# hlesmqh/WS3D

Measured on AMD Instinct MI355X. Metric: KITTI scenes/sec (16384 pts) Stage-1 RPN fwd, 1/2/4/8 GPU; FPS+group HBM GB/s, higher is better.
Workload: dtype f32

## Files before the change

include/ws3d_ops.h:

```cpp
#ifndef WS3D_OPS_H
#define WS3D_OPS_H

#include <stddef.h>
#include <stdint.h>

#ifdef __cplusplus
extern "C" {
#endif

#define WS3D_OK 0
#define WS3D_E_INVALID (-1)
#define WS3D_E_LAUNCH (-2)
#define WS3D_E_WORKSPACE (-3)
#define WS3D_E_UNSUPPORTED (-4)

#if defined(__GNUC__)
#define WS3D_API __attribute__((visibility("default")))
#else
#define WS3D_API
#endif

typedef void *ws3d_stream_t;

#define WS3D_ABI_VERSION 6
// ... 57 lines not shown
                  int32_t *idx, const void *sorted_known, ws3d_stream_t stream);

WS3D_API int ws3d_three_nn_weights(long rows, const float *dist2, float *weight, ws3d_stream_t stream);
WS3D_API int ws3d_three_nn_w(int b, int n, int m, const float *unknown, const float *known, float *dist2, int32_t *idx, float *weight,
                             const void *sorted_known, ws3d_stream_t stream);
WS3D_API int ws3d_three_nn_wq(int b, int n, int m, const float *unknown, const float *known, float *dist2, int32_t *idx, float *weight,
                              const void *sorted_known, const void *sorted_unknown, ws3d_stream_t stream);
WS3D_API int ws3d_three_nn_jobs(int b, int njobs, const int *n, const int *m, const float *const *unknown, const void *const *sorted_known,
                                float *const *dist2, int32_t *const *idx, float *const *weight, const void *const *sorted_unknown,
                                ws3d_stream_t stream);

WS3D_API int ws3d_pool_nsample(long rows, int nsample, const float *x, float *out, uint8_t *arg, ws3d_stream_t stream);
WS3D_API int ws3d_pool_nsample_grad(long rows, int nsample, const float *grad_out, const uint8_t *arg, float *grad_x,
                                    ws3d_stream_t stream);

WS3D_API int ws3d_gemm_pool(long rows, int nsample, int k_dim, int o_dim, const float *x_rows, const float *wt,
                            const float *bias, int relu, float *out, int out_stride, const int32_t *gate, long gate_limit, ws3d_stream_t stream);

WS3D_API int ws3d_gather_gemm(int b, int n, int m, int nsample, int c_feat, int o_dim, const float *feats, const float *xyz,
                     const float *new_xyz, const int32_t *nbr, const float *wt, const float *bias, int relu, float *out,
                     ws3d_stream_t stream);

WS3D_API int ws3d_gather_gemm2(int b, int n, int m, int nsample, int c_feat, int o1, int o2, const float *feats, const float *xyz,
                      const float *new_xyz, const int32_t *nbr, const float *w1t, const float *b1, int relu1, const float *w2t,
                      const float *b2, int relu2, float *out, ws3d_stream_t stream);

WS3D_API int ws3d_pgather_gemm2(int b, int n, int m, int nsample, int o1, int o2, const float *pmat, int p_stride, const float *xyz,
                       const float *new_xyz, const int32_t *nbr, const float *w1x, const float *b1, int relu1,
                       const float *w2t, const float *b2, int relu2, float *out, const int32_t *gate, long gate_limit, ws3d_stream_t stream);
WS3D_API int ws3d_pgather_rows(int b, int n, int m, int nsample, int o1, const float *pmat, int p_stride, const float *xyz, const float *new_xyz,
                      const int32_t *nbr, const float *w1x, const float *b1, int relu1, float *out, ws3d_stream_t stream);

WS3D_API int ws3d_qinterp_rows(int b, int n, int m, int o, const float *q, const int32_t *idx, const float *weight, const float *lin,
                      const float *skip, int c1, const float *wb, const float *bias, int relu, float *out, ws3d_stream_t stream);


WS3D_API int ws3d_compact_pairs(long centres, int nsample, const int32_t *nbr, int32_t *rowc, int32_t *rowsrc, int32_t *total, ws3d_stream_t stream);
WS3D_API int ws3d_compact_pairs_count(long centres, int nsample, const int32_t *nbr, int32_t *cnt, ws3d_stream_t stream);
WS3D_API int ws3d_compact_pairs_rows(long centres, int nsample, const int32_t *nbr, const int32_t *cnt, const int32_t *incl, int32_t *rowc,
                            int32_t *rowsrc, int32_t *total, ws3d_stream_t stream);
WS3D_API int ws3d_pgather_gemm2_compact(int b, int n, int m, long max_rows, int o1, int o2, const float *pmat, int p_stride, const float *xyz,
                               const float *new_xyz, const int32_t *rowc, const int32_t *rowsrc, const int32_t *total, const float *w1x,
                               const float *b1, int relu1, const float *w2t, const float *b2, int relu2, float *out, long limit, ws3d_stream_t stream);
WS3D_API int ws3d_pgather_gemm3_compact(int b, int n, int m, long max_rows, int o1, int o2, int o3, const float *pmat, int p_stride, const float *xyz,
                               const float *new_xyz, const int32_t *rowc, const int32_t *rowsrc, const int32_t *total, const float *w1x,
                               const float *b1, int relu1, const float *w2t, const float *b2, int relu2, const float *w3t, const float *b3,
                               float *out, int out_stride, long limit, ws3d_stream_t stream);
WS3D_API int ws3d_gemm_pool_compact(long max_rows, int k_dim, int o_dim, const float *x_rows, const int32_t *rowc, const int32_t *total,
                           const float *wt, const float *bias, float *out, int out_stride, long limit, ws3d_stream_t stream);
typedef struct ws3d_compact_mlp_args {
    int b, n, m;
    long max_rows;
    int o1, o2, o3;
    const float *pmat;
    int p_stride;
    const float *xyz, *new_xyz;
    const int32_t *rowc, *rowsrc, *total;
    const float *w1x, *b1;
    int relu1;
    const float *w2t, *b2;
    int relu2;
    const float *w3t, *b3;
    float *mid;
    float *out;
    int out_stride;
    long limit;
} ws3d_compact_mlp_args;
WS3D_API int ws3d_compact_mlp_pair(int kind, const ws3d_compact_mlp_args *scale0, const ws3d_compact_mlp_args *scale1, ws3d_stream_t stream);
WS3D_API int ws3d_chain_mlp3_ticket_ints(void);
WS3D_API size_t ws3d_chain_mlp3_blob_floats(int o2);
WS3D_API int ws3d_chain_mlp3_pack(const ws3d_compact_mlp_args *scale, float *blob, ws3d_stream_t stream);
WS3D_API int ws3d_chain_mlp3(const ws3d_compact_mlp_args *scale0, const ws3d_compact_mlp_args *scale1, const float *blob0, const float *blob1,
                             int32_t *ticket, int workgroups, ws3d_stream_t stream);

WS3D_API int ws3d_sa_mlp3_pool_compact(int b, int n, int m, long max_rows, int c1, int c2, int c3, const float *xyz, const float *new_xyz,
                              const float *feat, const int32_t *rowc, const int32_t *rowsrc, const int32_t *total, const float *w1t,
                              const float *b1, const float *w2t, const float *b2, const float *w3t, const float *b3, float *out,
                              int out_stride, long limit, ws3d_stream_t stream);

WS3D_API int ws3d_sa_mlp3_pool_lists(int b, int n, int m, int nsample, int c1, int c2, int c3, const float *xyz, const float *new_xyz,
                            const float *feat, const int32_t *nbr, const float *w1t, const float *b1, const float *w2t, const float *b2,
                            const float *w3t, const float *b3, int relu3, float *out, int out_stride, const int32_t *gate, long gate_limit,
                            ws3d_stream_t stream);

WS3D_API int ws3d_interp_gemm(int b, int n, int m, int c2, int c1, int o_dim, const float *known_feats, const float *unknown_feats,
                     const int32_t *idx, const float *weight, const float *wt, const float *bias, int relu, float *out,
                     ws3d_stream_t stream);

WS3D_API size_t ws3d_conv1x1_wgrad_workspace_bytes(int b, int o, int c, long l);
WS3D_API int ws3d_conv1x1_wgrad(int b, int o, int c, long l, const float *grad_out, const float *x, float *grad_w,
                                void *workspace, size_t workspace_bytes, ws3d_stream_t stream);

WS3D_API size_t ws3d_bn_workspace_bytes(int b, int c, long l);
WS3D_API int ws3d_bn_relu_train_fwd(int b, int c, long l, const float *x, const float *gamma, const float *beta, float eps,
                                    float momentum, int relu, float *running_mean, float *running_var,
                                    int64_t *num_batches_tracked, float *y, float *save_mean, float *save_invstd,
                                    void *workspace, size_t workspace_bytes, ws3d_stream_t stream);
WS3D_API int ws3d_bn_relu_train_bwd(int b, int c, long l, const float *x, const float *dy, const float *gamma,
                                    const float *beta, const float *save_mean, const float *save_invstd, int relu, float *dx,
                                    float *dgamma, float *dbeta, void *workspace, size_t workspace_bytes, ws3d_stream_t stream);

WS3D_API int ws3d_three_interpolate(int b, int c, int m, int n, const float *points, const int32_t *idx,
                           const float *weight, float *out, ws3d_stream_t stream);

WS3D_API int ws3d_three_interpolate_grad(int b, int c, int n, int m, const float *grad_out,
                                const int32_t *idx, const float *weight, float *grad_points,
                                ws3d_stream_t stream);

WS3D_API size_t ws3d_scatter_workspace_bytes(int b, int c, int n_targets, long slots_per_scene);
WS3D_API int ws3d_group_points_grad_det(int b, int c, int n, int npoints, int nsample, const float *grad_out,
                                        const int32_t *idx, float *grad_points, void *workspace,
                                        size_t workspace_bytes, ws3d_stream_t stream);
WS3D_API int ws3d_three_interpolate_grad_det(int b, int c, int n, int m, const float *grad_out, const int32_t *idx,
                                             const float *weight, float *grad_points, void *workspace,
                                             size_t workspace_bytes, ws3d_stream_t stream);

WS3D_API int ws3d_bias_act_inplace(int b, int o_ch, long l, int relu, float *y, const float *bias,
                                   ws3d_stream_t stream);

WS3D_API int ws3d_rowmax_bias_act(int b, int o_ch, long m, int s, int relu, const float *y, const float *bias,
                                  float *out, ws3d_stream_t stream);

WS3D_API int ws3d_query_and_group_nlc(int b, int n, int m, int c, float radius, int nsample, int use_xyz,
                                      const float *xyz, const float *new_xyz, const float *features_nlc,
                                      int32_t *idx_out, float *out_nlc, const void *sorted, ws3d_stream_t stream);
WS3D_API int ws3d_three_interpolate_nlc(int b, int c, int m, int n, const float *feats_nlc, const int32_t *idx,
                                        const float *weight, float *out_nlc, int out_stride, ws3d_stream_t stream);
WS3D_API int ws3d_rowmax_rows(long rows_out, int ns, int o_ch, const float *y, float *out, int out_stride,
                              ws3d_stream_t stream);

WS3D_API int ws3d_sa_mlp3_pool(long rows, int nsample, int c1, int c2, int c3, const float *x_rows4,
                               const float *w1t, const float *b1, const float *w2t, const float *b2,
                               const float *w3t, const float *b3, int relu3, float *out, int out_stride,
                               ws3d_stream_t stream);

WS3D_API int ws3d_mlp2_rows(long rows, int k_dim, int o1, int o2, const float *x_rows, const float *w1t, const float *b1, int relu1,
                   const float *w2t, const float *b2, int relu2, float *out, int *ticket, ws3d_stream_t stream);

WS3D_API size_t ws3d_rpn_heads_blob_bytes(int o2);
WS3D_API int ws3d_rpn_heads_pack(int o2, const float *w1t, const float *b1, int relu1, const float *w2t, const float *b2, int relu2, void *blob,
                        ws3d_stream_t stream);
WS3D_API int ws3d_rpn_heads(long rows, const float *x_rows, int heads, const void *blob_cls, float *out_cls, int *ticket_cls, int o2_reg,
                   const void *blob_reg, float *out_reg, int *ticket_reg, int workgroups, ws3d_stream_t stream);

WS3D_API size_t ws3d_gemm_rows_pack_bytes(int k_dim, int n_dim);
WS3D_API int ws3d_gemm_rows_pack(int k_dim, int n_dim, const float *wt, void *pack, ws3d_stream_t stream);
WS3D_API int ws3d_gemm_rows_split(long rows, int k_dim, int n_dim, const float *a, const void *pack, const float *bias, int relu, float *out,
                         ws3d_stream_t stream);

WS3D_API int ws3d_qinterp_gemm(int b, int n, int m, int c, int o_dim, const float *q, const int32_t *idx, const float *weight, const float *lin,
                      const float *skip, int c1, const float *wb, const float *b1, int relu1, const float *w2t, const float *b2, int relu2,
                      float *out, ws3d_stream_t stream);


WS3D_API int ws3d_boxes_overlap_bev(int num_a, const float *boxes_a, int num_b, const float *boxes_b,
                           float *ans, ws3d_stream_t stream);

WS3D_API int ws3d_boxes_iou_bev(int num_a, const float *boxes_a, int num_b, const float *boxes_b,
                       float *ans, ws3d_stream_t stream);

WS3D_API int ws3d_boxes_iou3d_paired(int n, const float *boxes_a, const float *boxes_b, float *overlap_bev, float *iou2d, float *iou3d,
                                     ws3d_stream_t stream);

WS3D_API int ws3d_nms_mask(int boxes_num, const float *boxes, float thresh, int normal, int full_grid,
                  uint64_t *mask, ws3d_stream_t stream);

WS3D_API size_t ws3d_nms_workspace_bytes(int boxes_num);
WS3D_API int ws3d_nms(int boxes_num, const float *boxes, float thresh, int normal, int max_keep,
                      void *workspace, size_t workspace_bytes, int64_t *keep, int32_t *num_keep,
                      ws3d_stream_t stream);

WS3D_API int ws3d_nms_batched(int batch, int boxes_num, const float *boxes, float thresh, int normal,
                              int max_keep, void *workspace, size_t workspace_bytes, int64_t *keep,
                              int32_t *num_keep, ws3d_stream_t stream);


WS3D_API int ws3d_radius_nms_batched(int batch, int n, const float *centers, float radius, int max_keep,
                                     void *workspace, size_t workspace_bytes, int64_t *keep,
                                     int32_t *num_keep, ws3d_stream_t stream);

WS3D_API int ws3d_topk_sorted(int b, int n, int k, const float *scores, float *out_scores, int64_t *out_idx,
                              ws3d_stream_t stream);
WS3D_API size_t ws3d_topk_workspace_bytes(int b, int n);
WS3D_API int ws3d_topk_sorted_ws(int b, int n, int k, const float *scores, float *out_scores, int64_t *out_idx, void *workspace,
                                 size_t workspace_bytes, ws3d_stream_t stream);
WS3D_API int ws3d_topk_sorted_sigmoid(int b, int n, int k, const float *logits, float *out_scores, int64_t *out_idx, ws3d_stream_t stream);
WS3D_API int ws3d_topk_sorted_sigmoid_ws(int b, int n, int k, const float *logits, float *out_scores, int64_t *out_idx, void *workspace,
                                         size_t workspace_bytes, ws3d_stream_t stream);

WS3D_API int ws3d_decode_center_boxes(int b, int n, int bins, float loc_scope, float loc_bin_size, float h, float w,
                                      float l, const float *xyz, const float *rpn_reg, float *boxes,
                                      ws3d_stream_t stream);

WS3D_API int ws3d_gather_boxes_bev(int b, int n, int top, const float *box, const int64_t *order, float *box_sorted, float *bev,
                          ws3d_stream_t stream);
WS3D_API int ws3d_decode_gather_boxes_bev(int b, int n, int top, int bins, float loc_scope, float loc_bin_size, float h, float w, float l,
                                          const float *xyz, const float *rpn_reg, const int64_t *order, float *box_sorted, float *bev,
                                          ws3d_stream_t stream);
WS3D_API int ws3d_select_proposals(int b, int top, int keep_stride, int k, const float *box_sorted, const float *scores_sorted,
                          const int64_t *keep, const int32_t *num, float extra_width, float *boxes_out, float *scores_out,
                          int64_t *count, float *pooled_boxes, ws3d_stream_t stream);
WS3D_API int ws3d_select_proposals_packed(int b, int top, int keep_stride, int k, const float *box_sorted, const float *scores_sorted,
                                          const int64_t *keep, const int32_t *num, float extra_width, float *boxes_out, float *scores_out,
                                          int64_t *count, float *pooled_boxes, float *packed, ws3d_stream_t stream);
WS3D_API int ws3d_select_proposals_send(int b, int top, int keep_stride, int k, const float *box_sorted, const float *scores_sorted,
                                        const int64_t *keep, const int32_t *num, float extra_width, float *boxes_out, float *scores_out,
                                        int64_t *count, float *pooled_boxes, float *send, long send_stride, ws3d_stream_t stream);
WS3D_API int ws3d_split_points_clear(long rows, int c, const float *pc, float *xyz, float *feats, void *clear, size_t clear_bytes,
                                     ws3d_stream_t stream);


WS3D_API int ws3d_roipool3d(int batch_size, int pts_num, int boxes_num, int feature_in_len,
                   int sampled_pts_num, const float *xyz, const float *boxes3d,
                   const float *pts_feature, float *pooled_features, int32_t *pooled_empty_flag,
                   int32_t *pts_idx, ws3d_stream_t stream);
WS3D_API int ws3d_roipool3d_fill(int batch_size, int pts_num, int boxes_num, int feature_in_len,
                   int sampled_pts_num, const float *xyz, const float *boxes3d,
                   const float *pts_feature, float *pooled_features, int32_t *pooled_empty_flag,
                   int32_t *pts_idx, ws3d_stream_t stream);

WS3D_API size_t ws3d_roipool3d_workspace_bytes(int batch_size, int pts_num);
WS3D_API int ws3d_roipool3d_ws(int batch_size, int pts_num, int boxes_num, int feature_in_len, int sampled_pts_num, const float *xyz,
                               const float *boxes3d, const float *pts_feature, float *pooled_features, int32_t *pooled_empty_flag,
                               int32_t *pts_idx, int fill, void *workspace, size_t workspace_bytes, ws3d_stream_t stream);


WS3D_API int ws3d_pts_in_boxes3d(int boxes_num, int pts_num, const float *pts, const float *boxes3d,
                        int64_t *flag, ws3d_stream_t stream);


WS3D_API int ws3d_instance_clouds(int batch, int pts_num, int centres_num, int feat_len, int sampled_pts_num, float radius, int mask_mode,
                                  float mask_thresh, const float *pts, const float *score, const float *feats, const float *centres,
                                  const int32_t *num, float *cloud, float *cloud_feats, int32_t *count, int32_t *pts_idx,
                                  ws3d_stream_t stream);
WS3D_API int ws3d_instance_clouds_count(int batch, int pts_num, int centres_num, float radius, const float *pts, const float *centres,
                                        const int32_t *num, int32_t *count, ws3d_stream_t stream);
WS3D_API int ws3d_instance_clouds_emit(int batch, int pts_num, int centres_num, int feat_len, float radius, int mask_mode, float mask_thresh,
                                       const float *pts, const float *score, const float *feats, const float *centres, const int32_t *num,
                                       const int64_t *offsets, float *rows, float *row_feats, int32_t *row_idx, ws3d_stream_t stream);


WS3D_API int ws3d_click_prepare(int batch, int pts_num, int clicks_num, int side, const float *offsets, float gauss_height, float gauss_status,
                                float gauss_cov, float centre_y, const float *pts, const float *clicks, const int32_t *num, float *score,
                                float *cand, int32_t *cand_num, ws3d_stream_t stream);



WS3D_API int ws3d_kitti_overlaps(int metric, int criterion, int frames, long max_pairs, const int32_t *gt_off, const int32_t *dt_off,
                                 const int64_t *out_off, const double *dt_boxes, const double *gt_boxes, double *out,
                                 ws3d_stream_t stream);

WS3D_API int ws3d_kitti_collect_scores(int frames, int max_dt, const int32_t *gt_off, const int32_t *dt_off, const int64_t *out_off,
                                       const double *overlaps, const int32_t *ignored_gt, const int32_t *ignored_dt,
                                       const double *dt_score, double min_overlap, double *tp_score, int32_t *tp_flag,
                                       ws3d_stream_t stream);

WS3D_API size_t ws3d_kitti_count_workspace_bytes(int frames, int num_thresh);
WS3D_API int ws3d_kitti_count(int metric, int frames, int max_dt, int num_thresh, const double *thresholds, const int32_t *gt_off,
                              const int32_t *dt_off, const int32_t *dc_off, const int64_t *out_off, const double *overlaps,
                              const int32_t *ignored_gt, const int32_t *ignored_dt, const double *dt_score, const double *dt_alpha,
                              const double *gt_alpha, const double *dt_bbox, const double *dc_bbox, double min_overlap, int compute_aos,
                              void *workspace, size_t workspace_bytes, double *pr, ws3d_stream_t stream);


WS3D_API int ws3d_stage2_embed(long rows, int pts_per_cloud, const float *pts, const float *box_ce, float extend, const float *wx0,
                               const float *bx0, const float *wx1, const float *bx1, const float *wf0, const float *bf0, const float *wf1,
                               const float *bf1, const float *wm, const float *bm, float *xyz_out, float *feat, ws3d_stream_t stream);
WS3D_API int ws3d_stage2_boxes(int rows, int loc_bins, int head_bins, float loc_scope, float h, float w, float l, const float *rcnn_reg,
                               float *pred_boxes3d, float *box_ce, ws3d_stream_t stream);
WS3D_API int ws3d_stage2_select(int batch, int slots, float cls_thresh, float iou_thresh, const float *size_window, float ground_y,
                                const float *box_ce, const float *rcnn_ref, const float *rcnn_cls, const float *rcnn_iou, const float *center,
                                const int32_t *num, float *boxes, int32_t *keep, float *key, ws3d_stream_t stream);

WS3D_API int ws3d_stage2_rcnn_loss(int rows, int loc_bins, int head_bins, float loc_scope, float h, float w, float l, const float *rcnn_cls,
                                   const float *rcnn_reg, const float *pred_boxes3d, const float *gt_boxes, const float *cls, float *vals,
                                   int32_t *counts, float *grad_cls, float *grad_reg, ws3d_stream_t stream);
WS3D_API int ws3d_stage2_ioun_loss(int rows, const float *rcnn_iou, const float *rcnn_ref, const float *pred_boxes3d, const float *refined_box,
                                   const float *gt_boxes, const float *cls, float *vals, int32_t *counts, float *grad_iou, float *grad_ref,
                                   ws3d_stream_t stream);

WS3D_API int ws3d_rpn_center_labels(int batch, int n, int kmax, int pts_stride, float gauss_height, float gauss_status, double gauss_cov,
                                    const float *pts, const float *centres, const int32_t *count, float *cls_label, float *reg_label,
                                    ws3d_stream_t stream);
WS3D_API size_t ws3d_rpn_loss_workspace_bytes(int rows);
WS3D_API int ws3d_rpn_loss(int rows, int bins, double loc_scope, double loc_bin_size, double alpha, double gamma, double weight_cls,
                           double weight_reg, const float *rpn_cls, const float *rpn_reg, const float *cls_label, const float *reg_label,
                           float *vals, int32_t *counts, float *grad_cls, float *grad_reg, void *workspace, size_t workspace_bytes,
                           ws3d_stream_t stream);

#ifdef __cplusplus
}
#endif
#endif
```

ws3d_amd/_lib.py:

```python
from __future__ import annotations

import ctypes as C
import os

_HERE = os.path.dirname(os.path.abspath(__file__))
DIST_MODE = int(os.environ.get("WS3D_DIST_MODE", "0") or 0)
LIB_PATH = os.environ.get("WS3D_HIP_LIB") or os.path.join(
    _HERE, "libws3d_hip.so" if DIST_MODE == 0 else "libws3d_hip_dm%d.so" % DIST_MODE)

E_INVALID, E_LAUNCH, E_WORKSPACE, E_UNSUPPORTED = -1, -2, -3, -4
ABI_VERSION = 6

_vp = C.c_void_p
_i = C.c_int
_f = C.c_float
_sz = C.c_size_t

class CompactMlpArgs(C.Structure):
    _fields_ = [("b", _i), ("n", _i), ("m", _i), ("max_rows", C.c_long), ("o1", _i), ("o2", _i), ("o3", _i), ("pmat", _vp), ("p_stride", _i),
                ("xyz", _vp), ("new_xyz", _vp), ("rowc", _vp), ("rowsrc", _vp), ("total", _vp), ("w1x", _vp), ("b1", _vp), ("relu1", _i),
                ("w2t", _vp), ("b2", _vp), ("relu2", _i), ("w3t", _vp), ("b3", _vp), ("mid", _vp), ("out", _vp), ("out_stride", _i), ("limit", C.c_long)]


SIGNATURES = {
    "ws3d_abi_version": (_i, []),
    "ws3d_tune": (_i, [_i, _i]),
    "ws3d_dist_mode": (_i, []),
    "ws3d_last_error": (C.c_char_p, []),
    "ws3d_device_info": (_i, [C.c_char_p, _i, C.POINTER(_i), C.POINTER(_i)]),
    "ws3d_furthest_point_sampling": (_i, [_i, _i, _i, _vp, _vp, _vp, _vp]),
    "ws3d_furthest_point_sampling_gather": (_i, [_i, _i, _i, _vp, _vp, _vp, _vp, _vp]),
    "ws3d_furthest_point_sampling_nested": (_i, [_i, _i, _i, _vp, _vp, _vp, _vp]),
    "ws3d_furthest_point_sampling_nested_chain": (_i, [_i, _i, _i, _vp, _vp, _vp, _vp, _vp]),
    "ws3d_gather_points": (_i, [_i, _i, _i, _i, _vp, _vp, _vp, _vp]),
    "ws3d_gather_points_grad": (_i, [_i, _i, _i, _i, _vp, _vp, _vp, _vp]),
    "ws3d_ball_query": (_i, [_i, _i, _i, _f, _i, _vp, _vp, _vp, _vp, _vp]),
    "ws3d_ball_query_fill": (_i, [_i, _i, _i, _f, _i, _vp, _vp, _vp, _vp, _vp]),
    "ws3d_ball_query_pairs": (_i, [_i, _i, _i, _f, _i, _vp, _vp, _vp, _vp, _vp, _vp, _vp, _vp]),
    "ws3d_ball_query_pairs2": (_i, [_i, _i, _i, _vp, _vp, _vp, C.c_float, _i, _vp, _vp, _vp, _vp, C.c_float, _i, _vp, _vp, _vp, _vp, _vp]),
    "ws3d_sorted_points_bytes": (_sz, [_i, _i]),
    "ws3d_sort_points_x": (_i, [_i, _i, _vp, _vp, _vp]),
    "ws3d_sort_points_xz": (_i, [_i, _i, _vp, _vp, _vp]),
    "ws3d_sort_points_grid": (_i, [_i, _i, _vp, _vp, _vp]),
    "ws3d_sort_points_jobs": (_i, [_i, _i, _vp, _vp, _vp, _vp, _vp]),
    "ws3d_group_points": (_i, [_i, _i, _i, _i, _i, _vp, _vp, _vp, _vp]),
    "ws3d_group_points_grad": (_i, [_i, _i, _i, _i, _i, _vp, _vp, _vp, _vp]),
    "ws3d_query_and_group": (_i, [_i, _i, _i, _i, _f, _i, _i, _vp, _vp, _vp, _vp, _vp, _vp, _vp]),
    "ws3d_three_nn": (_i, [_i, _i, _i, _vp, _vp, _vp, _vp, _vp, _vp]),
    "ws3d_three_interpolate": (_i, [_i, _i, _i, _i, _vp, _vp, _vp, _vp, _vp]),
    "ws3d_three_interpolate_grad": (_i, [_i, _i, _i, _i, _vp, _vp, _vp, _vp, _vp]),
    "ws3d_bn_workspace_bytes": (C.c_size_t, [_i, _i, C.c_long]),
    "ws3d_bn_relu_train_fwd": (_i, [_i, _i, C.c_long, _vp, _vp, _vp, C.c_float, C.c_float, _i, _vp, _vp, _vp, _vp, _vp, _vp,
                                    _vp, C.c_size_t, _vp]),
    "ws3d_bn_relu_train_bwd": (_i, [_i, _i, C.c_long, _vp, _vp, _vp, _vp, _vp, _vp, _i, _vp, _vp, _vp, _vp, C.c_size_t, _vp]),
    "ws3d_conv1x1_wgrad_workspace_bytes": (C.c_size_t, [_i, _i, _i, C.c_long]),
    "ws3d_conv1x1_wgrad": (_i, [_i, _i, _i, C.c_long, _vp, _vp, _vp, _vp, C.c_size_t, _vp]),
    "ws3d_gemm_pool": (_i, [C.c_long, _i, _i, _i, _vp, _vp, _vp, _i, _vp, _i, _vp, C.c_long, _vp]),
    "ws3d_pool_nsample": (_i, [C.c_long, _i, _vp, _vp, _vp, _vp]),
    "ws3d_pool_nsample_grad": (_i, [C.c_long, _i, _vp, _vp, _vp, _vp]),
    "ws3d_scatter_workspace_bytes": (C.c_size_t, [_i, _i, _i, C.c_long]),
    "ws3d_group_points_grad_det": (_i, [_i, _i, _i, _i, _i, _vp, _vp, _vp, _vp, C.c_size_t, _vp]),
    "ws3d_three_interpolate_grad_det": (_i, [_i, _i, _i, _i, _vp, _vp, _vp, _vp, _vp, C.c_size_t, _vp]),
    "ws3d_query_and_group_nlc": (_i, [_i, _i, _i, _i, _f, _i, _i, _vp, _vp, _vp, _vp, _vp, _vp, _vp]),
    "ws3d_three_interpolate_nlc": (_i, [_i, _i, _i, _i, _vp, _vp, _vp, _vp, _i, _vp]),
    "ws3d_rowmax_rows": (_i, [C.c_long, _i, _i, _vp, _vp, _i, _vp]),
    "ws3d_sa_mlp3_pool": (_i, [C.c_long, _i, _i, _i, _i, _vp, _vp, _vp, _vp, _vp, _vp, _vp, _i, _vp, _i, _vp]),
    "ws3d_qinterp_gemm": (_i, [_i, _i, _i, _i, _i, _vp, _vp, _vp, _vp, _vp, _i, _vp, _vp, _i, _vp, _vp, _i, _vp, _vp]),
    "ws3d_mlp2_rows": (_i, [C.c_long, _i, _i, _i, _vp, _vp, _vp, _i, _vp, _vp, _i, _vp, _vp, _vp]),
    "ws3d_rpn_heads_blob_bytes": (_sz, [_i]),
    "ws3d_rpn_heads_pack": (_i, [_i, _vp, _vp, _i, _vp, _vp, _i, _vp, _vp]),
    "ws3d_rpn_heads": (_i, [C.c_long, _vp, _i, _vp, _vp, _vp, _i, _vp, _vp, _vp, _i, _vp]),
    "ws3d_gemm_rows_pack_bytes": (_sz, [_i, _i]),
    "ws3d_gemm_rows_pack": (_i, [_i, _i, _vp, _vp, _vp]),
    "ws3d_gemm_rows_split": (_i, [C.c_long, _i, _i, _vp, _vp, _vp, _i, _vp, _vp]),
    "ws3d_decode_center_boxes": (_i, [_i, _i, _i, _f, _f, _f, _f, _f, _vp, _vp, _vp, _vp]),
    "ws3d_topk_sorted": (_i, [_i, _i, _i, _vp, _vp, _vp, _vp]),
    "ws3d_topk_workspace_bytes": (C.c_size_t, [_i, _i]),
    "ws3d_topk_sorted_ws": (_i, [_i, _i, _i, _vp, _vp, _vp, _vp, C.c_size_t, _vp]),
    "ws3d_topk_sorted_sigmoid": (_i, [_i, _i, _i, _vp, _vp, _vp, _vp]),
    "ws3d_topk_sorted_sigmoid_ws": (_i, [_i, _i, _i, _vp, _vp, _vp, _vp, C.c_size_t, _vp]),
    "ws3d_three_nn_weights": (_i, [C.c_long, _vp, _vp, _vp]),
    "ws3d_three_nn_w": (_i, [_i, _i, _i, _vp, _vp, _vp, _vp, _vp, _vp, _vp]),
    "ws3d_three_nn_wq": (_i, [_i, _i, _i, _vp, _vp, _vp, _vp, _vp, _vp, _vp, _vp]),
    "ws3d_three_nn_jobs": (_i, [_i, _i, _vp, _vp, _vp, _vp, _vp, _vp, _vp, _vp, _vp]),
    "ws3d_bias_act_inplace": (_i, [_i, _i, C.c_long, _i, _vp, _vp, _vp]),
    "ws3d_rowmax_bias_act": (_i, [_i, _i, C.c_long, _i, _i, _vp, _vp, _vp, _vp]),
    "ws3d_boxes_overlap_bev": (_i, [_i, _vp, _i, _vp, _vp, _vp]),
    "ws3d_boxes_iou_bev": (_i, [_i, _vp, _i, _vp, _vp, _vp]),
    "ws3d_boxes_iou3d_paired": (_i, [_i, _vp, _vp, _vp, _vp, _vp, _vp]),
    "ws3d_nms_mask": (_i, [_i, _vp, _f, _i, _i, _vp, _vp]),
    "ws3d_nms_workspace_bytes": (_sz, [_i]),
    "ws3d_nms": (_i, [_i, _vp, _f, _i, _i, _vp, _sz, _vp, _vp, _vp]),
    "ws3d_nms_batched": (_i, [_i, _i, _vp, _f, _i, _i, _vp, _sz, _vp, _vp, _vp]),
    "ws3d_radius_nms_batched": (_i, [_i, _i, _vp, _f, _i, _vp, _sz, _vp, _vp, _vp]),
    "ws3d_gather_gemm": (_i, [_i, _i, _i, _i, _i, _i, _vp, _vp, _vp, _vp, _vp, _vp, _i, _vp, _vp]),
    "ws3d_gather_gemm2": (_i, [_i, _i, _i, _i, _i, _i, _i, _vp, _vp, _vp, _vp, _vp, _vp, _i, _vp, _vp, _i, _vp, _vp]),
    "ws3d_pgather_gemm2": (_i, [_i, _i, _i, _i, _i, _i, _vp, _i, _vp, _vp, _vp, _vp, _vp, _i, _vp, _vp, _i, _vp, _vp, C.c_long, _vp]),
    "ws3d_pgather_rows": (_i, [_i, _i, _i, _i, _i, _vp, _i, _vp, _vp, _vp, _vp, _vp, _i, _vp, _vp]),
    "ws3d_qinterp_rows": (_i, [_i, _i, _i, _i, _vp, _vp, _vp, _vp, _vp, _i, _vp, _vp, _i, _vp, _vp]),
    "ws3d_compact_pairs": (_i, [C.c_long, _i, _vp, _vp, _vp, _vp, _vp]),
    "ws3d_compact_pairs_count": (_i, [C.c_long, _i, _vp, _vp, _vp]),
    "ws3d_compact_pairs_rows": (_i, [C.c_long, _i, _vp, _vp, _vp, _vp, _vp, _vp, _vp]),
    "ws3d_pgather_gemm2_compact": (_i, [_i, _i, _i, C.c_long, _i, _i, _vp, _i, _vp, _vp, _vp, _vp, _vp, _vp, _vp, _i, _vp, _vp, _i, _vp, C.c_long, _vp]),
    "ws3d_pgather_gemm3_compact": (_i, [_i, _i, _i, C.c_long, _i, _i, _i, _vp, _i, _vp, _vp, _vp, _vp, _vp, _vp, _vp, _i, _vp, _vp, _i, _vp, _vp, _vp, _i, C.c_long, _vp]),
    "ws3d_gemm_pool_compact": (_i, [C.c_long, _i, _i, _vp, _vp, _vp, _vp, _vp, _vp, _i, C.c_long, _vp]),
    "ws3d_compact_mlp_pair": (_i, [_i, C.POINTER(CompactMlpArgs), C.POINTER(CompactMlpArgs), _vp]),
    "ws3d_chain_mlp3_ticket_ints": (_i, []),
    "ws3d_chain_mlp3_blob_floats": (_sz, [_i]),
    "ws3d_chain_mlp3_pack": (_i, [C.POINTER(CompactMlpArgs), _vp, _vp]),
    "ws3d_chain_mlp3": (_i, [C.POINTER(CompactMlpArgs), C.POINTER(CompactMlpArgs), _vp, _vp, _vp, _i, _vp]),
    "ws3d_sa_mlp3_pool_compact": (_i, [_i, _i, _i, C.c_long, _i, _i, _i, _vp, _vp, _vp, _vp, _vp, _vp, _vp, _vp, _vp, _vp, _vp, _vp, _vp, _i, C.c_long, _vp]),
    "ws3d_sa_mlp3_pool_lists": (_i, [_i, _i, _i, _i, _i, _i, _i, _vp, _vp, _vp, _vp, _vp, _vp, _vp, _vp, _vp, _vp, _i, _vp, _i, _vp, C.c_long, _vp]),
    "ws3d_interp_gemm": (_i, [_i, _i, _i, _i, _i, _i, _vp, _vp, _vp, _vp, _vp, _vp, _i, _vp, _vp]),
    "ws3d_gather_boxes_bev": (_i, [_i, _i, _i, _vp, _vp, _vp, _vp, _vp]),
    "ws3d_select_proposals": (_i, [_i, _i, _i, _i, _vp, _vp, _vp, _vp, _f, _vp, _vp, _vp, _vp, _vp]),
    "ws3d_decode_gather_boxes_bev": (_i, [_i, _i, _i, _i, _f, _f, _f, _f, _f, _vp, _vp, _vp, _vp, _vp, _vp]),
    "ws3d_select_proposals_packed": (_i, [_i, _i, _i, _i, _vp, _vp, _vp, _vp, _f, _vp, _vp, _vp, _vp, _vp, _vp]),
    "ws3d_select_proposals_send": (_i, [_i, _i, _i, _i, _vp, _vp, _vp, _vp, _f, _vp, _vp, _vp, _vp, _vp, C.c_long, _vp]),
    "ws3d_split_points_clear": (_i, [C.c_long, _i, _vp, _vp, _vp, _vp, C.c_size_t, _vp]),
    "ws3d_roipool3d": (_i, [_i, _i, _i, _i, _i, _vp, _vp, _vp, _vp, _vp, _vp, _vp]),
    "ws3d_roipool3d_fill": (_i, [_i, _i, _i, _i, _i, _vp, _vp, _vp, _vp, _vp, _vp, _vp]),
    "ws3d_roipool3d_workspace_bytes": (C.c_size_t, [_i, _i]),
    "ws3d_roipool3d_ws": (_i, [_i, _i, _i, _i, _i, _vp, _vp, _vp, _vp, _vp, _vp, _i, _vp, C.c_size_t, _vp]),
    "ws3d_pts_in_boxes3d": (_i, [_i, _i, _vp, _vp, _vp, _vp]),
    "ws3d_instance_clouds": (_i, [_i, _i, _i, _i, _i, _f, _i, _f, _vp, _vp, _vp, _vp, _vp, _vp, _vp, _vp, _vp, _vp]),
    "ws3d_instance_clouds_count": (_i, [_i, _i, _i, _f, _vp, _vp, _vp, _vp, _vp]),
    "ws3d_instance_clouds_emit": (_i, [_i, _i, _i, _i, _f, _i, _f, _vp, _vp, _vp, _vp, _vp, _vp, _vp, _vp, _vp, _vp]),
    "ws3d_click_prepare": (_i, [_i, _i, _i, _i, _vp, _f, _f, _f, _f, _vp, _vp, _vp, _vp, _vp, _vp, _vp]),
    "ws3d_kitti_overlaps": (_i, [_i, _i, _i, C.c_long, _vp, _vp, _vp, _vp, _vp, _vp, _vp]),
    "ws3d_kitti_collect_scores": (_i, [_i, _i, _vp, _vp, _vp, _vp, _vp, _vp, _vp, C.c_double, _vp, _vp, _vp]),
    "ws3d_kitti_count_workspace_bytes": (_sz, [_i, _i]),
    "ws3d_kitti_count": (_i, [_i, _i, _i, _i, _vp, _vp, _vp, _vp, _vp, _vp, _vp, _vp, _vp, _vp, _vp, _vp, _vp, C.c_double, _i, _vp,
                              _sz, _vp, _vp]),
    "ws3d_stage2_embed": (_i, [C.c_long, _i, _vp, _vp, _f] + [_vp] * 10 + [_vp, _vp, _vp]),
    "ws3d_stage2_boxes": (_i, [_i, _i, _i, _f, _f, _f, _f, _vp, _vp, _vp, _vp]),
    "ws3d_stage2_select": (_i, [_i, _i, _f, _f, C.POINTER(_f), _f, _vp, _vp, _vp, _vp, _vp, _vp, _vp, _vp, _vp, _vp]),
    "ws3d_stage2_rcnn_loss": (_i, [_i, _i, _i, _f, _f, _f, _f] + [_vp] * 9 + [_vp]),
    "ws3d_stage2_ioun_loss": (_i, [_i] + [_vp] * 10 + [_vp]),
    "ws3d_rpn_center_labels": (_i, [_i, _i, _i, _i, _f, _f, C.c_double] + [_vp] * 5 + [_vp]),
    "ws3d_rpn_loss_workspace_bytes": (_sz, [_i]),
    "ws3d_rpn_loss": (_i, [_i, _i] + [C.c_double] * 6 + [_vp] * 8 + [_vp, _sz, _vp]),
}


class Ws3dError(RuntimeError):
    pass


_lib = None


def load() -> C.CDLL:
    global _lib
    if _lib is not None:
        return _lib
    if not os.path.exists(LIB_PATH):
        raise Ws3dError(
            f"{LIB_PATH} is missing: the MI355X HIP library has not been built "
            "(run `python -m ws3d_amd.build`).  ws3d_amd has no CPU fallback.")
    import torch
    try:
        lib = C.CDLL(LIB_PATH)
    except OSError as e:
        raise Ws3dError(f"cannot load {LIB_PATH}: {e}") from e
    for name, (res, args) in SIGNATURES.items():
        fn = getattr(lib, name)
        fn.restype = res
        fn.argtypes = args
    if lib.ws3d_abi_version() != ABI_VERSION:
        raise Ws3dError(f"{LIB_PATH} exports ABI version {lib.ws3d_abi_version()}, this package binds version {ABI_VERSION}: "
                        "rebuild it (`python -m ws3d_amd.build`)")
    if not os.environ.get("WS3D_HIP_LIB") and lib.ws3d_dist_mode() != DIST_MODE:
        raise Ws3dError(f"{LIB_PATH} was built with WS3D_DIST_MODE={lib.ws3d_dist_mode()}, expected {DIST_MODE}: rebuild it")
    _lib = lib
    return lib


def check(rc: int, what: str = "") -> None:
    if rc != 0:
        msg = load().ws3d_last_error()
        raise Ws3dError(f"{what or 'ws3d'} failed (rc={rc}): {msg.decode() if msg else ''}")
```

ws3d_amd/build.py:

```python
from __future__ import annotations

import argparse
import concurrent.futures as cf
import glob
import os
import shutil
import subprocess
import sys

HERE = os.path.dirname(os.path.abspath(__file__))
CSRC = os.path.join(HERE, "csrc")
OBJ = os.path.join(CSRC, "build")
LIB = os.path.join(HERE, "libws3d_hip.so")
DIST_MODES = (0, 1, 2)


def lib_path(dist_mode: int = 0) -> str:
    return LIB if dist_mode == 0 else os.path.join(HERE, "libws3d_hip_dm%d.so" % dist_mode)
ARCH = "gfx950"
SOURCES = ["core.hip", "fps.hip", "fps_v3.hip", "fps_bucket.hip", "fps_nested.hip", "ballquery_group.hip", "interpolate.hip", "roipool3d.hip", "iou3d.hip", "proposals.hip", "scatter_det.hip", "sa_mlp.hip", "bn_relu.hip", "gemm_pool.hip", "conv_wgrad.hip", "chain_mlp.hip", "rpn_heads.hip", "gemm_rows.hip", "kitti_eval.hip", "instance_clouds.hip", "click.hip", "stage2.hip", "stage2_loss.hip", "rpn_targets.hip"]
CXXFLAGS = ["-O3", "-std=c++17", "-fPIC", "-ffp-contract=off", "-fno-fast-math",
            "-fvisibility=hidden", "-Wall", "-Wno-unused-function"]


def hipcc() -> str:
    for cand in (os.environ.get("HIPCC"), shutil.which("hipcc"), "/opt/rocm/bin/hipcc"):
        if cand and os.path.exists(cand):
            return cand
    raise RuntimeError("hipcc not found (looked at $HIPCC, PATH, /opt/rocm/bin)")


def _deps(src: str):
    return [src, *glob.glob(os.path.join(CSRC, "*.h")), os.path.join(HERE, "..", "include", "ws3d_ops.h"),
            os.path.join(CSRC, "exports.map"), os.path.abspath(__file__)]


def _compile(src: str, force: bool, verbose: bool, dist_mode: int = 0) -> str:
    path = os.path.join(CSRC, src)
    obj = os.path.join(OBJ if dist_mode == 0 else OBJ + "_dm%d" % dist_mode, os.path.splitext(src)[0] + ".o")
    if not force and os.path.exists(obj) and all(
            os.path.getmtime(obj) >= os.path.getmtime(d) for d in _deps(path)):
        return obj
    cmd = [hipcc(), f"--offload-arch={ARCH}", *CXXFLAGS, f"-DWS3D_DIST_MODE={dist_mode}", *os.environ.get("WS3D_EXTRA_DEFS", "").split(), "-c", path, "-o", obj]
    if verbose:
        print(" ".join(cmd), flush=True)
    r = subprocess.run(cmd, capture_output=True, text=True)
    if r.returncode != 0:
        raise RuntimeError(f"hipcc failed for {src}:\n{r.stdout}\n{r.stderr}")
    if verbose and r.stderr.strip():
        print(r.stderr)
    return obj


def build(force: bool = False, verbose: bool = False, dist_mode: int = 0) -> str:
    LIB = lib_path(dist_mode)
    os.makedirs(OBJ if dist_mode == 0 else OBJ + "_dm%d" % dist_mode, exist_ok=True)
    with cf.ThreadPoolExecutor(max_workers=min(len(SOURCES), os.cpu_count() or 4, 16)) as ex:
        objs = list(ex.map(lambda s: _compile(s, force, verbose, dist_mode), SOURCES))
    if force or not os.path.exists(LIB) or any(os.path.getmtime(o) > os.path.getmtime(LIB) for o in objs):
        cmd = [hipcc(), f"--offload-arch={ARCH}", "-shared", "-fPIC", "-Wl,--version-script=" + os.path.join(CSRC, "exports.map"), "-o", LIB, *objs]
        if verbose:
            print(" ".join(cmd), flush=True)
        r = subprocess.run(cmd, capture_output=True, text=True)
        if r.returncode != 0:
            raise RuntimeError(f"link failed:\n{r.stdout}\n{r.stderr}")
    return LIB


def rebuild_one(src: str, verbose: bool = False) -> str:
    _compile(src, True, verbose)
    objs = [os.path.join(OBJ, os.path.splitext(s_)[0] + ".o") for s_ in SOURCES]
    missing = [o for o in objs if not os.path.exists(o)]
    if missing:
        return build(False, verbose)
    cmd = [hipcc(), f"--offload-arch={ARCH}", "-shared", "-fPIC", "-Wl,--version-script=" + os.path.join(CSRC, "exports.map"), "-o", LIB, *objs]
    r = subprocess.run(cmd, capture_output=True, text=True)
    if r.returncode != 0:
        raise RuntimeError(f"link failed:\n{r.stdout}\n{r.stderr}")
    return LIB


if __name__ == "__main__":
    ap = argparse.ArgumentParser()
    ap.add_argument("--force", action="store_true")
    ap.add_argument("--verbose", action="store_true")
    ap.add_argument("--dist-mode", type=int, default=0, choices=DIST_MODES)
    ap.add_argument("--all-dist-modes", action="store_true")
    ap.add_argument("--only", default=None, help="recompile this one source (forced) and relink")
    a = ap.parse_args()
    if a.only:
        print(rebuild_one(a.only, a.verbose))
        sys.exit(0)
    for dm in (DIST_MODES if a.all_dist_modes else (a.dist_mode,)):
        print(build(a.force, a.verbose, dm))
    sys.exit(0)
```

ws3d_amd/compat.py:

```python
from __future__ import annotations

import sys
import types

import os

import torch

from . import _lib
from ._lib import Ws3dError, check


def _dev(*tensors):
    dev = None
    for t in tensors:
        if t is None:
            continue
        if not t.is_cuda:
            raise Ws3dError("ws3d_amd ops need HIP ('cuda') tensors; there is no CPU fallback")
        if not t.is_contiguous():
            raise Ws3dError("ws3d_amd ops need contiguous tensors (the reference asserts the same)")
        if dev is None:
            dev = t.device
        elif t.device != dev:
# ... 355 lines not shown
    b, c = x.size(0), x.size(1)
    l = x.numel() // max(b * c, 1)
    y = torch.empty_like(x)
    mean = torch.empty((c,), dtype=torch.float32, device=dev)
    invstd = torch.empty((c,), dtype=torch.float32, device=dev)
    lib = _lib.load()
    nbytes = lib.ws3d_bn_workspace_bytes(b, c, l)
    ws = torch.empty((nbytes + 7) // 8, dtype=torch.float64, device=dev)
    with _on(dev):
        check(lib.ws3d_bn_relu_train_fwd(b, c, l, _p(x), _p(gamma), _p(beta), float(eps), float(momentum), int(bool(relu)),
                                         _p(running_mean), _p(running_var), _p(num_batches_tracked), _p(y), _p(mean), _p(invstd), _p(ws), nbytes,
                                         _stream()), "bn_relu_train_fwd")
    return y, mean, invstd


def bn_relu_train_bwd(x, dy, gamma, beta, save_mean, save_invstd, relu=True):
    dev = _dev(x, dy, gamma, beta, save_mean, save_invstd)
    _f32(x, "x"); _f32(dy, "dy")
    b, c = x.size(0), x.size(1)
    l = x.numel() // max(b * c, 1)
    dx = torch.empty_like(x)
    dgamma = torch.empty((c,), dtype=torch.float32, device=dev)
    dbeta = torch.empty((c,), dtype=torch.float32, device=dev)
    lib = _lib.load()
    nbytes = lib.ws3d_bn_workspace_bytes(b, c, l)
    ws = torch.empty((nbytes + 7) // 8, dtype=torch.float64, device=dev)
    with _on(dev):
        check(lib.ws3d_bn_relu_train_bwd(b, c, l, _p(x), _p(dy), _p(gamma), _p(beta), _p(save_mean), _p(save_invstd),
                                         int(bool(relu)), _p(dx), _p(dgamma), _p(dbeta), _p(ws), nbytes, _stream()),
              "bn_relu_train_bwd")
    return dx, dgamma, dbeta


def conv1x1_wgrad(grad_out, x, shape=None):
    dev = _dev(grad_out, x)
    _f32(grad_out, "grad_out"); _f32(x, "x")
    b, o, c = x.size(0), grad_out.size(1), x.size(1)
    l = x.numel() // max(b * c, 1)
    if grad_out.numel() != b * o * l:
        raise Ws3dError("conv1x1_wgrad: grad_out and x disagree in shape")
    gw = torch.empty((o, c) if shape is None else tuple(shape), dtype=torch.float32, device=dev)
    lib = _lib.load()
    nbytes = lib.ws3d_conv1x1_wgrad_workspace_bytes(b, o, c, l)
    ws = torch.empty((nbytes + 3) // 4, dtype=torch.float32, device=dev)
    with _on(dev):
        check(lib.ws3d_conv1x1_wgrad(b, o, c, l, _p(grad_out), _p(x), _p(gw), _p(ws), nbytes, _stream()), "conv1x1_wgrad")
    return gw


def _gate(gate):
    if gate is None:
        return None, 0
    total, limit = gate
    return total.data_ptr(), int(limit)


def gemm_pool(x_rows, wt, bias, relu, nsample, out, col0=0, gate=None):
    dev = _dev(x_rows, wt, bias)
    _f32(x_rows, "x_rows"); _f32(wt, "wt")
    rows, k = x_rows.shape
    o = wt.size(1)
    if rows % 64 or rows // 64 > 65535 or o % 64 or k % 4 or nsample not in (16, 32) or wt.size(0) != k:
        return False
    view = out[:, col0:col0 + o]
    with _on(dev):
        check(_lib.load().ws3d_gemm_pool(rows, nsample, k, o, _p(x_rows), _p(wt), _p(bias), int(bool(relu)), view.data_ptr(),
                                         out.size(1), *_gate(gate), _stream()), "gemm_pool")
    return True


def gather_gemm(feats, xyz, new_xyz, nbr, wt_feat_then_xyz, bias, relu):
    dev = _dev(feats, xyz, new_xyz, nbr, wt_feat_then_xyz)
    _f32(feats, "feats"); _f32(xyz, "xyz"); _f32(new_xyz, "new_xyz"); _i32(nbr, "nbr"); _f32(wt_feat_then_xyz, "wt")
    B, N, C = feats.shape
    M, ns = nbr.size(1), nbr.size(2)
    O = wt_feat_then_xyz.size(1)
    rows = B * M * ns
    if C % 4 or O % 64 or rows % 64 or rows // 64 > 65535 or wt_feat_then_xyz.size(0) != C + 3 or not feats.is_contiguous():
        return None
    out = torch.empty((rows, O), dtype=torch.float32, device=dev)
    with _on(dev):
        check(_lib.load().ws3d_gather_gemm(B, N, M, ns, C, O, _p(feats), _p(xyz), _p(new_xyz), _p(nbr), _p(wt_feat_then_xyz), _p(bias),
                                           int(bool(relu)), _p(out), _stream()), "gather_gemm")
    return out


def gather_gemm2(feats, xyz, new_xyz, nbr, w1t_feat_then_xyz, b1, relu1, w2t, b2, relu2):
    dev = _dev(feats, xyz, new_xyz, nbr, w1t_feat_then_xyz, w2t)
    _f32(feats, "feats"); _f32(xyz, "xyz"); _f32(new_xyz, "new_xyz"); _i32(nbr, "nbr"); _f32(w1t_feat_then_xyz, "w1t"); _f32(w2t, "w2t")
    B, N, C = feats.shape
    M, ns = nbr.size(1), nbr.size(2)
    O1, O2 = w1t_feat_then_xyz.size(1), w2t.size(1)
    rows = B * M * ns
    if (C % 4 or O1 not in (64, 128, 256) or O2 % 4 or rows % 64 or w1t_feat_then_xyz.size(0) != C + 3 or w2t.size(0) != O1 or
            not feats.is_contiguous() or not w2t.is_contiguous() or not w1t_feat_then_xyz.is_contiguous()):
        return None
    out = torch.empty((rows, O2), dtype=torch.float32, device=dev)
    with _on(dev):
        check(_lib.load().ws3d_gather_gemm2(B, N, M, ns, C, O1, O2, _p(feats), _p(xyz), _p(new_xyz), _p(nbr), _p(w1t_feat_then_xyz), _p(b1),
                                            int(bool(relu1)), _p(w2t), _p(b2), int(bool(relu2)), _p(out), _stream()), "gather_gemm2")
    return out


def pgather_gemm2(pmat, col0, o1, xyz, new_xyz, nbr, w1x, b1, relu1, w2t, b2, relu2, out=None, gate=None):
    dev = _dev(pmat, xyz, new_xyz, nbr, w1x, w2t)
    _f32(pmat, "pmat"); _f32(xyz, "xyz"); _f32(new_xyz, "new_xyz"); _i32(nbr, "nbr"); _f32(w1x, "w1x"); _f32(w2t, "w2t")
    B, N = xyz.size(0), xyz.size(1)
    M, ns = nbr.size(1), nbr.size(2)
    O2 = w2t.size(1)
    if (o1 not in (64, 128) or O2 % 4 or (M * ns) % 64 or pmat.dim() != 2 or pmat.size(0) != B * N or pmat.stride(1) != 1 or
            col0 < 0 or col0 + o1 > pmat.size(1) or tuple(w1x.shape) != (3, o1) or w2t.size(0) != o1 or not w1x.is_contiguous() or not w2t.is_contiguous()):
        return None
    if out is None:
        out = torch.empty((B * M * ns, O2), dtype=torch.float32, device=dev)
    elif tuple(out.shape) != (B * M * ns, O2) or not out.is_contiguous():
        raise ValueError("pgather_gemm2: out must be a contiguous (B*M*ns, O2) tensor")
    with _on(dev):
        check(_lib.load().ws3d_pgather_gemm2(B, N, M, ns, o1, O2, pmat.data_ptr() + 4 * col0, pmat.stride(0), _p(xyz), _p(new_xyz), _p(nbr), _p(w1x), _p(b1),
                                             int(bool(relu1)), _p(w2t), _p(b2), int(bool(relu2)), _p(out), *_gate(gate), _stream()), "pgather_gemm2")
    return out


def pgather_rows(pmat, col0, o1, xyz, new_xyz, nbr, w1x, b1, relu1):
    dev = _dev(pmat, xyz, new_xyz, nbr, w1x)
    _f32(pmat, "pmat"); _f32(xyz, "xyz"); _f32(new_xyz, "new_xyz"); _i32(nbr, "nbr"); _f32(w1x, "w1x")
    B, N = xyz.size(0), xyz.size(1)
    M, ns = nbr.size(1), nbr.size(2)
    if (o1 % 4 or col0 % 4 or pmat.dim() != 2 or pmat.size(0) != B * N or pmat.stride(1) != 1 or pmat.stride(0) % 4 or col0 < 0 or
            col0 + o1 > pmat.size(1) or tuple(w1x.shape) != (3, o1) or not w1x.is_contiguous() or pmat.data_ptr() % 16):
        return None
    out = torch.empty((B * M * ns, o1), dtype=torch.float32, device=dev)
    with _on(dev):
        check(_lib.load().ws3d_pgather_rows(B, N, M, ns, o1, pmat.data_ptr() + 4 * col0, pmat.stride(0), _p(xyz), _p(new_xyz), _p(nbr), _p(w1x), _p(b1),
                                            int(bool(relu1)), _p(out), _stream()), "pgather_rows")
    return out


def qinterp_rows(q, idx, weight, lin=None, skip=None, wb=None, bias=None, relu=True):
    dev = _dev(q, idx, weight)
    _f32(q, "q"); _i32(idx, "idx"); _f32(weight, "weight")
    B, M, O = q.shape
    N = idx.size(1)
    c1 = 0 if skip is None else skip.size(2)
    if (O % 4 or not q.is_contiguous() or (lin is None and c1 > 4) or (lin is not None and (tuple(lin.shape) != (B * N, O) or not lin.is_contiguous())) or
            (lin is None and c1 > 0 and (wb is None or tuple(wb.shape) != (c1, O) or not wb.is_contiguous() or not skip.is_contiguous()))):
        return None
    out = torch.empty((B * N, O), dtype=torch.float32, device=dev)
    with _on(dev):
        check(_lib.load().ws3d_qinterp_rows(B, N, M, O, _p(q), _p(idx), _p(weight), _p(lin), _p(skip), c1, _p(wb), _p(bias), int(bool(relu)), _p(out),
                                            _stream()), "qinterp_rows")
    return out


def qinterp_gemm(q, idx, weight, w2t, b2, relu2, lin=None, skip=None, wb=None, bias=None, relu=True):
    dev = _dev(q, idx, weight, w2t)
    _f32(q, "q"); _i32(idx, "idx"); _f32(weight, "weight"); _f32(w2t, "w2t")
    B, M, C = q.shape
    N = idx.size(1)
    O = w2t.size(1)
    c1 = 0 if skip is None else skip.size(2)
    if ((B * N) % 64 or C % 16 or O % 128 or w2t.size(0) != C or not q.is_contiguous() or not w2t.is_contiguous() or not idx.is_contiguous() or
            not weight.is_contiguous() or (lin is None and c1 > 4) or (lin is not None and (tuple(lin.shape) != (B * N, C) or not lin.is_contiguous())) or
            (lin is None and c1 > 0 and (wb is None or tuple(wb.shape) != (c1, C) or not wb.is_contiguous() or not skip.is_contiguous()))):
        return None
    out = torch.empty((B * N, O), dtype=torch.float32, device=dev)
    with _on(dev):
        check(_lib.load().ws3d_qinterp_gemm(B, N, M, C, O, _p(q), _p(idx), _p(weight), _p(lin), _p(skip), c1, _p(wb), _p(bias), int(bool(relu)), _p(w2t),
                                            _p(b2), int(bool(relu2)), _p(out), _stream()), "qinterp_gemm")
    return out


def compact_pairs(nbr, ordered=False):
    if not ordered:
        dev = _dev(nbr)
        _i32(nbr, "nbr")
        B, M, ns = nbr.shape
        rowc = torch.empty(B * M * ns, dtype=torch.int32, device=dev)
        rowsrc = torch.empty(B * M * ns, dtype=torch.int32, device=dev)
        total = torch.zeros(1, dtype=torch.int32, device=dev)
        with _on(dev):
            check(_lib.load().ws3d_compact_pairs(B * M, ns, _p(nbr), _p(rowc), _p(rowsrc), _p(total), _stream()), "compact_pairs")
        return rowc, rowsrc, total
    dev = _dev(nbr)
    _i32(nbr, "nbr")
    B, M, ns = nbr.shape
    centres = B * M
    cnt = torch.empty(centres, dtype=torch.int32, device=dev)
    rowc = torch.empty(centres * ns, dtype=torch.int32, device=dev)
    rowsrc = torch.empty(centres * ns, dtype=torch.int32, device=dev)
    total = torch.empty(1, dtype=torch.int32, device=dev)
    with _on(dev):
        lib = _lib.load()
        check(lib.ws3d_compact_pairs_count(centres, ns, _p(nbr), _p(cnt), _stream()), "compact_pairs_count")
        incl = torch.cumsum(cnt, dim=0, dtype=torch.int32)
        check(lib.ws3d_compact_pairs_rows(centres, ns, _p(nbr), _p(cnt), _p(incl), _p(rowc), _p(rowsrc), _p(total), _stream()), "compact_pairs_rows")
    return rowc, rowsrc, total


def pgather_gemm2_compact(pmat, col0, o1, xyz, new_xyz, pairs, w1x, b1, relu1, w2t, b2, relu2, limit=-1):
    rowc, rowsrc, total = pairs
    dev = _dev(pmat, xyz, new_xyz, rowc, w1x, w2t)
    _f32(pmat, "pmat"); _f32(xyz, "xyz"); _f32(new_xyz, "new_xyz"); _f32(w1x, "w1x"); _f32(w2t, "w2t")
    B, N = xyz.size(0), xyz.size(1)
    M = new_xyz.size(1)
    O2 = w2t.size(1)
    rows = rowc.numel()
    if (o1 not in (64, 128, 256) or O2 % 4 or pmat.dim() != 2 or pmat.size(0) != B * N or pmat.stride(1) != 1 or col0 < 0 or col0 + o1 > pmat.size(1) or
            tuple(w1x.shape) != (3, o1) or w2t.size(0) != o1 or not w1x.is_contiguous() or not w2t.is_contiguous()):
        return None
    out = torch.empty((rows, O2), dtype=torch.float32, device=dev)
    with _on(dev):
        check(_lib.load().ws3d_pgather_gemm2_compact(B, N, M, rows, o1, O2, pmat.data_ptr() + 4 * col0, pmat.stride(0), _p(xyz), _p(new_xyz), _p(rowc),
                                                     _p(rowsrc), _p(total), _p(w1x), _p(b1), int(bool(relu1)), _p(w2t), _p(b2), int(bool(relu2)), _p(out),
                                                     int(limit), _stream()), "pgather_gemm2_compact")
    return out


def pgather_gemm3_compact(pmat, col0, o1, xyz, new_xyz, pairs, w1x, b1, relu1, w2t, b2, relu2, w3t, b3, out2d, col_offset, limit=-1, max_lds=160 * 1024):
    rowc, rowsrc, total = pairs
    dev = _dev(pmat, xyz, new_xyz, rowc, w1x, w2t, w3t, out2d)
    _f32(pmat, "pmat"); _f32(xyz, "xyz"); _f32(new_xyz, "new_xyz"); _f32(w1x, "w1x"); _f32(w2t, "w2t"); _f32(w3t, "w3t"); _f32(out2d, "out2d")
    B, N = xyz.size(0), xyz.size(1)
    M = new_xyz.size(1)
    O2, O3 = w2t.size(1), w3t.size(1)
    rows = rowc.numel()
    lds = 4 * ((o1 + (O2 + 15) // 16 * 16) * 65 + 2 * 16 * 64)
    if (o1 not in (64, 128) or O2 % 4 or O3 % 128 or lds > min(max_lds, 160 * 1024 - 1024) or pmat.dim() != 2 or pmat.size(0) != B * N or pmat.stride(1) != 1 or
            col0 < 0 or col0 + o1 > pmat.size(1) or tuple(w1x.shape) != (3, o1) or w2t.size(0) != o1 or w3t.size(0) != O2 or not w1x.is_contiguous() or
            not w2t.is_contiguous() or not w3t.is_contiguous() or out2d.dim() != 2 or out2d.stride(1) != 1 or col_offset < 0 or col_offset + O3 > out2d.size(1)):
        return False
    with _on(dev):
        check(_lib.load().ws3d_pgather_gemm3_compact(B, N, M, rows, o1, O2, O3, pmat.data_ptr() + 4 * col0, pmat.stride(0), _p(xyz), _p(new_xyz), _p(rowc),
                                                     _p(rowsrc), _p(total), _p(w1x), _p(b1), int(bool(relu1)), _p(w2t), _p(b2), int(bool(relu2)), _p(w3t), _p(b3),
                                                     out2d.data_ptr() + 4 * col_offset, out2d.stride(0), int(limit), _stream()), "pgather_gemm3_compact")
    return True


def gemm_pool_compact(x_rows, pairs, wt, bias, out2d, col_offset, limit=-1):
    rowc, rowsrc, total = pairs
    dev = _dev(x_rows, rowc, wt, out2d)
    _f32(x_rows, "x_rows"); _f32(wt, "wt"); _f32(out2d, "out2d")
    rows, k = x_rows.shape
    o = wt.size(1)
    if (k % 4 or o % 64 or wt.size(0) != k or rows != rowc.numel() or not x_rows.is_contiguous() or not wt.is_contiguous() or out2d.dim() != 2 or
            out2d.stride(1) != 1 or col_offset < 0 or col_offset + o > out2d.size(1)):
        return False
    with _on(dev):
        check(_lib.load().ws3d_gemm_pool_compact(rows, k, o, _p(x_rows), _p(rowc), _p(total), _p(wt), _p(bias), out2d.data_ptr() + 4 * col_offset,
                                                 out2d.stride(0), int(limit), _stream()), "gemm_pool_compact")
    return True


def compact_mlp_pair(kind, scales, max_lds=160 * 1024, mids=None):
    import ctypes as C
    if len(scales) != 2 or scales[0]["o1"] != scales[1]["o1"]:
        return None if kind == 2 else False
    blocks, keep, outs = [], [], []
    for si, a in enumerate(scales):
        rowc, rowsrc, total = a["pairs"]
        pmat, xyz, new_xyz, w1x, w2t, w3t, out2d, o1, col0, col = a["pmat"], a["xyz"], a["new_xyz"], a["w1x"], a["w2t"], a["w3t"], a["out2d"], a["o1"], a["col0"], a["col_offset"]
        dev = _dev(pmat, xyz, new_xyz, rowc, w1x, w2t, w3t, out2d)
        for t_, nm in ((pmat, "pmat"), (xyz, "xyz"), (new_xyz, "new_xyz"), (w1x, "w1x"), (w2t, "w2t"), (w3t, "w3t"), (out2d, "out2d")):
            _f32(t_, nm)
        B, N, M = xyz.size(0), xyz.size(1), new_xyz.size(1)
        O2, O3 = w2t.size(1), w3t.size(1)
        rows = rowc.numel()
        lds3 = 4 * ((o1 + (O2 + 15) // 16 * 16) * 65 + 2 * 16 * 64)
        ok = (O2 % 4 == 0 and pmat.dim() == 2 and pmat.size(0) == B * N and pmat.stride(1) == 1 and col0 >= 0 and col0 + o1 <= pmat.size(1) and
              tuple(w1x.shape) == (3, o1) and w2t.size(0) == o1 and w3t.size(0) == O2 and w1x.is_contiguous() and w2t.is_contiguous() and w3t.is_contiguous() and
              out2d.dim() == 2 and out2d.stride(1) == 1 and col >= 0 and col + O3 <= out2d.size(1))
        if kind == 3:
            ok = ok and o1 in (64, 128) and O3 % 128 == 0 and lds3 <= min(max_lds, 160 * 1024 - 1024)
        elif kind == 2:
            ok = ok and o1 in (64, 128, 256)
        else:
            ok = ok and O3 % 64 == 0 and mids is not None and tuple(mids[si].shape) == (rows, O2) and mids[si].is_contiguous()
        if not ok:
            return None if kind == 2 else False
        mid = mids[si] if kind == 1 else (torch.empty((rows, O2), dtype=torch.float32, device=dev) if kind == 2 else None)
        outs.append(mid)
        keep.append((pmat, xyz, new_xyz, rowc, rowsrc, total, w1x, w2t, w3t, out2d, mid, a["b1"], a["b2"], a["b3"]))
        blocks.append(_lib.CompactMlpArgs(B, N, M, rows, o1, O2, O3, pmat.data_ptr() + 4 * col0, pmat.stride(0), _p(xyz), _p(new_xyz), _p(rowc), _p(rowsrc),
                                          _p(total), _p(w1x), _p(a["b1"]), int(bool(a["relu1"])), _p(w2t), _p(a["b2"]), int(bool(a["relu2"])), _p(w3t), _p(a["b3"]),
                                          _p(mid), out2d.data_ptr() + 4 * col, out2d.stride(0), -1))
    with _on(dev):
        rc = _lib.load().ws3d_compact_mlp_pair(int(kind), C.byref(blocks[0]), C.byref(blocks[1]), _stream())
    if rc == _lib.E_UNSUPPORTED:
        return None if kind == 2 else False
    check(rc, "compact_mlp_pair")
    return outs if kind == 2 else True


CHAIN_WORKGROUPS = 0
TUNE_KEYS = {"chain_wgs": 0, "mlp2_wgs": 1, "sa1_wgs": 2, "fp_wgs": 3, "pair_wgs": 4, "bq_wide_nw": 5}


def tune(name: str, value: int = -1) -> int:
    rc = _lib.load().ws3d_tune(TUNE_KEYS[name], int(value))
    if rc < 0:
        check(rc, "tune")
    return rc


_CHAIN_BLOBS = {}


def chain_ticket_ints() -> int:
    return int(_lib.load().ws3d_chain_mlp3_ticket_ints())


def _chain_blob(block, tensors, dev):
    import ctypes as C
    key = tuple((t.data_ptr(), t._version) if t is not None else None for t in tensors)
    hit = _CHAIN_BLOBS.get(key)
    if hit is None:
        n = int(_lib.load().ws3d_chain_mlp3_blob_floats(block.o2))
        blob = torch.empty(n, dtype=torch.float32, device=dev)
        with _on(dev):
            check(_lib.load().ws3d_chain_mlp3_pack(C.byref(block), _p(blob), _stream()), "chain_mlp3_pack")
# ... 898 lines not shown
```

ws3d_amd/csrc/gemm_pool.hip:

```cpp
#include <cstdlib>

#include "common.h"
#include "compact_pool.h"
#include "mfma_tile.h"

namespace ws3d {

template <int NS, int MB, int NB>
__global__ __launch_bounds__(256) void gemm_pool_big_kernel(int k_dim, int o_dim, const float *__restrict__ x,
                                                            const float *__restrict__ wt, const float *__restrict__ bias,
                                                            int relu, float *__restrict__ out, int out_stride, int xcd,
                                                            const int32_t *__restrict__ gate, long gate_limit) {
    if (gate && (long)*gate <= gate_limit) return;
    constexpr int TM = 64 * MB, TN = 64 * NB;
    __shared__ float xs[2][GP_KT][TM + 1];
    __shared__ __attribute__((aligned(16))) float ws[2][GP_KT][TN];
    const Wave w;
    long row_tile;
    int col_tile;
    gg_tile<false>(o_dim / TN, xcd, blockIdx.x, row_tile, col_tile);
    const long row0 = row_tile * TM;
    const int col0 = col_tile * TN;
    RowsA<MB> load_a;
    load_a.k_dim = k_dim;
#pragma unroll
    for (int i = 0; i < MB; ++i) load_a.p[i] = x + (row0 + (w.tid >> 2) + 64 * i) * (long)k_dim;
    floatx16 acc[MB][NB];
    mfma_k_loop<MB, NB, false>(w, acc, xs, ws, k_dim, load_a, wt, o_dim, col0);
#pragma unroll
    for (int i = 0; i < MB; ++i)
#pragma unroll
        for (int j = 0; j < NB; ++j)
            pool_rows<NS>(w, acc[i][j], bias, relu, out, out_stride, row0 + sub_row<MB>(w, i), col0 + sub_col<NB, false>(w, j) + w.l32);
}

struct GatherA {
    const float *frow, *prow, *crow;
    int c_feat;
    __device__ __forceinline__ GatherA(long r, int c_feat_, int n, int m, int ns, const float *__restrict__ feats, const float *__restrict__ xyz,
                                       const float *__restrict__ new_xyz, const int32_t *__restrict__ nbr) {
        const long cm = r / ns;
        const long b = cm / m;
        const int src = nbr[r];
        frow = feats + ((size_t)b * n + (size_t)src) * c_feat_;
        prow = xyz + ((size_t)b * n + (size_t)src) * 3;
        crow = new_xyz + (size_t)cm * 3;
        c_feat = c_feat_;
    }
    __device__ __forceinline__ float4 operator()(int, int k) const {
        if (k < c_feat) return *reinterpret_cast<const float4 *>(frow + k);
        if (k == c_feat) return make_float4(prow[0] - crow[0], prow[1] - crow[1], prow[2] - crow[2], 0.f);
        return f4_zero();
    }
};

__global__ __launch_bounds__(256) void gather_gemm_kernel(int c_feat, int o_dim, int n, int m, int ns, const float *__restrict__ feats,
                                                          const float *__restrict__ xyz, const float *__restrict__ new_xyz,
                                                          const int32_t *__restrict__ nbr, const float *__restrict__ wt,
                                                          const float *__restrict__ bias, int relu, float *__restrict__ out, int tps) {
    __shared__ float xs[2][GP_KT][GP_XS];
    __shared__ __attribute__((aligned(16))) float ws[2][GP_KT][64];
    const Wave w;
    long row_tile;
    int col_tile;
    gg_tile<true>(o_dim / 64, tps, blockIdx.x, row_tile, col_tile);
    const long row0 = row_tile * 64;
    const int col0 = col_tile * 64;
    const GatherA load_a(row0 + (w.tid >> 2), c_feat, n, m, ns, feats, xyz, new_xyz, nbr);
    floatx16 acc[1][1];
    mfma_k_loop<1, 1, false>(w, acc, xs, ws, c_feat + 3, load_a, wt, o_dim, col0);
    store_rows(w, acc[0][0], bias, relu, out, o_dim, row0 + w.wm * 32, col0 + w.bc);
}

template <int NB1>
__global__ __launch_bounds__(256) void gather_gemm2_kernel(int c_feat, int o2, int n, int m, int ns, const float *__restrict__ feats,
                                                           const float *__restrict__ xyz, const float *__restrict__ new_xyz,
                                                           const int32_t *__restrict__ nbr, const float *__restrict__ w1t,
                                                           const float *__restrict__ b1, int relu1, const float *__restrict__ w2t,
                                                           const float *__restrict__ b2, int relu2, float *__restrict__ out) {
    constexpr int O1 = NB1 * 64;
    extern __shared__ __attribute__((aligned(16))) float smem2[];
    auto &xs = *reinterpret_cast<float (*)[2][GP_KT][GP_XS]>(smem2);
    auto &w1s = *reinterpret_cast<float (*)[2][GP_KT][O1]>(smem2 + 2 * GP_KT * GP_XS);
    float *act = smem2, *w2s = smem2 + O1 * GP_XS;
    const Wave w;
    const long row0 = (long)blockIdx.x * 64;
    const GatherA load_a(row0 + (w.tid >> 2), c_feat, n, m, ns, feats, xyz, new_xyz, nbr);
    floatx16 acc1[1][NB1];
    mfma_k_loop<1, NB1, true>(w, acc1, xs, w1s, c_feat + 3, load_a, w1t, O1, 0);
#pragma unroll
    for (int j = 0; j < NB1; ++j) store_act(w, acc1[0][j], b1, relu1, act, j * 64 + w.bc);
    lds_layer<1>(w, act, O1 / GP_KT, w2t, O1, o2, w2s, 0, 1, [&](const floatx16 &acc, int col) __attribute__((always_inline)) {
        if (col < o2) store_rows(w, acc, b2, relu2, out, o2, row0 + w.wm * 32, col);
    });
}

template <int NB1>
__global__ __launch_bounds__(256) void pgather_gemm2_kernel(int o2, int n, int m, int ns, const float *__restrict__ pmat, int p_stride,
                                                            const float *__restrict__ xyz, const float *__restrict__ new_xyz,
                                                            const int32_t *__restrict__ nbr, const float *__restrict__ w1x,
                                                            const float *__restrict__ b1, int relu1, const float *__restrict__ w2t,
                                                            const float *__restrict__ b2, int relu2, float *__restrict__ out,
                                                            const int32_t *__restrict__ gate, long gate_limit) {
    if (gate && (long)*gate <= gate_limit) return;
    constexpr int O1 = NB1 * 64;
    extern __shared__ __attribute__((aligned(16))) float smem2[];
    float *act = smem2, *w2s = smem2 + O1 * GP_XS;
    const Wave w;
    const long row0 = (long)blockIdx.x * 64;
    const long scene = row0 / ((long)m * ns);
    ppoint_layer1<NB1>(w, [&](int tr) __attribute__((always_inline)) { return PairRow{scene, (row0 + tr) / ns, nbr[row0 + tr]}; }, n, pmat, p_stride, xyz, new_xyz, w1x, b1, relu1, act);
    lds_layer<1>(w, act, O1 / GP_KT, w2t, O1, o2, w2s, 0, 1, [&](const floatx16 &acc, int col) __attribute__((always_inline)) {
        if (col < o2) store_rows(w, acc, b2, relu2, out, o2, row0 + w.wm * 32, col);
    });
}

__global__ __launch_bounds__(256) void pgather_rows_kernel(long rows, int o1, int n, int m, int ns, const float *__restrict__ pmat, int p_stride,
                                                           const float *__restrict__ xyz, const float *__restrict__ new_xyz,
                                                           const int32_t *__restrict__ nbr, const float *__restrict__ w1x,
                                                           const float *__restrict__ b1, int relu1, float *__restrict__ out) {
    const int q4 = o1 >> 2;
    const long total = rows * q4;
    for (long e = (long)blockIdx.x * 256 + threadIdx.x; e < total; e += (long)gridDim.x * 256) {
        const long r = e / q4;
        const int c4 = (int)(e - r * q4) * 4;
        const long cm = r / ns, scene = cm / m;
        const int src = nbr[r];
        const float *pr = xyz + ((size_t)scene * n + (size_t)src) * 3, *cr = new_xyz + (size_t)cm * 3;
        const float dx = pr[0] - cr[0], dy = pr[1] - cr[1], dz = pr[2] - cr[2];
        const float4 pv = *reinterpret_cast<const float4 *>(pmat + ((size_t)scene * n + (size_t)src) * p_stride + c4);
        const float4 wx = *reinterpret_cast<const float4 *>(w1x + c4), wy = *reinterpret_cast<const float4 *>(w1x + o1 + c4),
                     wz = *reinterpret_cast<const float4 *>(w1x + 2 * o1 + c4);
        const float4 bv = b1 ? *reinterpret_cast<const float4 *>(b1 + c4) : make_float4(0.f, 0.f, 0.f, 0.f);
        float4 y;
        y.x = __builtin_fmaf(dz, wz.x, __builtin_fmaf(dy, wy.x, __builtin_fmaf(dx, wx.x, pv.x))) + bv.x;
        y.y = __builtin_fmaf(dz, wz.y, __builtin_fmaf(dy, wy.y, __builtin_fmaf(dx, wx.y, pv.y))) + bv.y;
        y.z = __builtin_fmaf(dz, wz.z, __builtin_fmaf(dy, wy.z, __builtin_fmaf(dx, wx.z, pv.z))) + bv.z;
        y.w = __builtin_fmaf(dz, wz.w, __builtin_fmaf(dy, wy.w, __builtin_fmaf(dx, wx.w, pv.w))) + bv.w;
        if (relu1) { y.x = y.x < 0.f ? 0.f : y.x; y.y = y.y < 0.f ? 0.f : y.y; y.z = y.z < 0.f ? 0.f : y.z; y.w = y.w < 0.f ? 0.f : y.w; }
        *reinterpret_cast<float4 *>(out + r * (long)o1 + c4) = y;
    }
}

__global__ __launch_bounds__(256) void pair_count_kernel(long centres, int ns, const int32_t *__restrict__ nbr, int32_t *__restrict__ cnt) {
    const long c = (long)blockIdx.x * 256 + threadIdx.x;
    if (c >= centres) return;
    const int32_t *row = nbr + c * ns;
    int k = 1, prev = row[0];
    for (int s2 = 1; s2 < ns; ++s2) { const int v = row[s2]; k += v > prev; prev = v; }
    cnt[c] = k;
}

__global__ __launch_bounds__(256) void pair_rows_kernel(long centres, int ns, const int32_t *__restrict__ nbr, const int32_t *__restrict__ cnt,
                                                        const int32_t *__restrict__ incl, int32_t *__restrict__ rowc, int32_t *__restrict__ rowsrc,
                                                        int32_t *__restrict__ total) {
    const long e = (long)blockIdx.x * 256 + threadIdx.x;
    if (e >= centres * ns) return;
// ... 30 lines not shown
        for (int s2 = 0; s2 < k; ++s2) { rowc[first + s2] = (int32_t)c; rowsrc[first + s2] = row[s2]; }
    }
}

struct CompactSrc {
    const int32_t *__restrict__ rowc, *__restrict__ rowsrc;
    long row0, T;
    int m;
    __device__ __forceinline__ PairRow operator()(int tr) const {
        const long t = min(row0 + tr, T - 1);
        const int cm = rowc[t];
        return PairRow{cm / m, cm, rowsrc[t]};
    }
};

template <int NB1>
__device__ __forceinline__ void pgather_gemm2_compact_body(const unsigned bx, const unsigned by, const unsigned gy, int o2, int n, int m,
                                                           const float *__restrict__ pmat, int p_stride,
                                                           const float *__restrict__ xyz, const float *__restrict__ new_xyz,
                                                           const int32_t *__restrict__ rowc, const int32_t *__restrict__ rowsrc,
                                                           const int32_t *__restrict__ total, const float *__restrict__ w1x,
                                                           const float *__restrict__ b1, int relu1, const float *__restrict__ w2t,
                                                           const float *__restrict__ b2, int relu2, float *__restrict__ out, long limit) {
    constexpr int O1 = NB1 * 64;
    const long T = *total;
    const long row0 = (long)bx * 64;
    if (row0 >= T || (limit >= 0 && T > limit)) return;
    extern __shared__ __attribute__((aligned(16))) float smem2[];
    float *act = smem2, *w2s = smem2 + O1 * GP_XS;
    const Wave w;
    ppoint_layer1<NB1>(w, CompactSrc{rowc, rowsrc, row0, T, m}, n, pmat, p_stride, xyz, new_xyz, w1x, b1, relu1, act);
    lds_layer<1>(w, act, O1 / GP_KT, w2t, O1, o2, w2s, (int)by, (int)gy, [&](const floatx16 &acc, int col) __attribute__((always_inline)) {
        if (col < o2) store_rows(w, acc, b2, relu2, out, o2, row0 + w.wm * 32, col, T);
    });
}

template <int NB1>
__global__ __launch_bounds__(256) void pgather_gemm2_compact_kernel(int o2, int n, int m, const float *__restrict__ pmat, int p_stride,
                                                                    const float *__restrict__ xyz, const float *__restrict__ new_xyz,
                                                                    const int32_t *__restrict__ rowc, const int32_t *__restrict__ rowsrc,
                                                                    const int32_t *__restrict__ total, const float *__restrict__ w1x,
                                                                    const float *__restrict__ b1, int relu1, const float *__restrict__ w2t,
                                                                    const float *__restrict__ b2, int relu2, float *__restrict__ out, long limit) {
    pgather_gemm2_compact_body<NB1>(blockIdx.x, blockIdx.y, gridDim.y, o2, n, m, pmat, p_stride, xyz, new_xyz, rowc, rowsrc, total, w1x, b1, relu1, w2t, b2,
                                    relu2, out, limit);
}

struct CompactMlpArgs {
    const float *pmat, *xyz, *new_xyz;
    const int32_t *rowc, *rowsrc, *total;
    const float *w1x, *b1, *w2t, *b2, *w3t, *b3;
    float *mid, *out;
    long limit;
    int o2, o3, n, m, p_stride, relu1, relu2, out_stride, gy, pad;
};

template <int NB1>
__global__ __launch_bounds__(256) void pgather_gemm2_compact_pair_kernel(const CompactMlpArgs a0, const CompactMlpArgs a1, const unsigned split,
                                                                         const unsigned total_x) {
    for (unsigned bx = blockIdx.x; bx < total_x; bx += gridDim.x) {
        const bool second = bx >= split;
        const CompactMlpArgs &a = second ? a1 : a0;
        if (blockIdx.y < (unsigned)a.gy)
            pgather_gemm2_compact_body<NB1>(second ? bx - split : bx, blockIdx.y, (unsigned)a.gy, a.o2, a.n, a.m, a.pmat, a.p_stride, a.xyz, a.new_xyz,
                                            a.rowc, a.rowsrc, a.total, a.w1x, a.b1, a.relu1, a.w2t, a.b2, a.relu2, a.mid, a.limit);
        __syncthreads();
    }
}

__device__ __forceinline__ void gemm_pool_compact_body(const unsigned bx, int k_dim, int o_dim, const float *__restrict__ x, const int32_t *__restrict__ rowc,
                                                       const int32_t *__restrict__ total, const float *__restrict__ wt,
                                                       const float *__restrict__ bias, float *__restrict__ out, int out_stride, long limit) {
    const long T = *total;
    const int col_tiles = o_dim / 64;
    const long row_tile = bx / col_tiles;
    const int col_tile = (int)(bx - row_tile * col_tiles);
    const long row0 = row_tile * 64;
    if (row0 >= T || (limit >= 0 && T > limit)) return;
    __shared__ float xs[2][GP_KT][GP_XS];
    __shared__ __attribute__((aligned(16))) float ws[2][GP_KT][64];
    const Wave w;
    const int col0 = col_tile * 64;
    const RowsA<1> load_a{{x + min(row0 + (w.tid >> 2), T - 1) * (long)k_dim}, k_dim};
    floatx16 acc[1][1];
    mfma_k_loop<1, 1, false>(w, acc, xs, ws, k_dim, load_a, wt, o_dim, col0);
    const int col = col0 + w.bc;
    int cen[16];
    compact_centres16(rowc, row0 + w.wm * 32 + 16 * w.kh, T, cen);
    compact_pool_atomic(acc[0][0], bias ? bias[col] : 0.f, cen, out + col, out_stride);
}

__global__ __launch_bounds__(256) void gemm_pool_compact_kernel(int k_dim, int o_dim, const float *__restrict__ x, const int32_t *__restrict__ rowc,
                                                                const int32_t *__restrict__ total, const float *__restrict__ wt,
                                                                const float *__restrict__ bias, float *__restrict__ out, int out_stride, long limit) {
    gemm_pool_compact_body(blockIdx.x, k_dim, o_dim, x, rowc, total, wt, bias, out, out_stride, limit);
}

__global__ __launch_bounds__(256) void gemm_pool_compact_pair_kernel(const CompactMlpArgs a0, const CompactMlpArgs a1, const unsigned split, const unsigned total_x) {
    for (unsigned bx = blockIdx.x; bx < total_x; bx += gridDim.x) {
        const bool second = bx >= split;
        const CompactMlpArgs &a = second ? a1 : a0;
        gemm_pool_compact_body(second ? bx - split : bx, a.o2, a.o3, a.mid, a.rowc, a.total, a.w3t, a.b3, a.out, a.out_stride, a.limit);
        __syncthreads();
    }
}

template <int NB1>
__device__ __forceinline__ void pgather_gemm3_compact_body(const unsigned bx, int o2, int o3, int n, int m, const float *__restrict__ pmat, int p_stride,
                                                           const float *__restrict__ xyz, const float *__restrict__ new_xyz,
                                                           const int32_t *__restrict__ rowc, const int32_t *__restrict__ rowsrc,
                                                           const int32_t *__restrict__ total, const float *__restrict__ w1x,
                                                           const float *__restrict__ b1, int relu1, const float *__restrict__ w2t,
                                                           const float *__restrict__ b2, int relu2, const float *__restrict__ w3t,
                                                           const float *__restrict__ b3, float *__restrict__ out, int out_stride, long limit) {
    constexpr int O1 = NB1 * 64;
    const long T = *total;
    const long row0 = (long)bx * 64;
    if (row0 >= T || (limit >= 0 && T > limit)) return;
    extern __shared__ __attribute__((aligned(16))) float smem2[];
    const int o2p = (o2 + GP_KT - 1) / GP_KT * GP_KT;
    float *act = smem2, *act2 = smem2 + O1 * GP_XS, *w2s = smem2 + (O1 + o2p) * GP_XS;
    const Wave w;
    int cidx[16];
    compact_centres16(rowc, row0 + w.wm * 32 + 16 * w.kh, T, cidx);
    ppoint_layer1<NB1>(w, CompactSrc{rowc, rowsrc, row0, T, m}, n, pmat, p_stride, xyz, new_xyz, w1x, b1, relu1, act);
    lds_layer<1>(w, act, O1 / GP_KT, w2t, O1, o2, w2s, 0, 1, [&](const floatx16 &acc, int col) __attribute__((always_inline)) {
        if (col < o2p) store_act(w, acc, b2, relu2, act2, col, o2);
    });
    lds_layer<2>(w, act2, o2p / GP_KT, w3t, o2, o3, smem2, 0, 1, [&](const floatx16 &acc, int col) __attribute__((always_inline)) {
        compact_pool_atomic(acc, b3 ? b3[col] : 0.f, cidx, out + col, out_stride);
    });
}

template <int NB1>
__global__ __launch_bounds__(256) void pgather_gemm3_compact_kernel(int o2, int o3, int n, int m, const float *__restrict__ pmat, int p_stride,
                                                                    const float *__restrict__ xyz, const float *__restrict__ new_xyz,
                                                                    const int32_t *__restrict__ rowc, const int32_t *__restrict__ rowsrc,
                                                                    const int32_t *__restrict__ total, const float *__restrict__ w1x,
                                                                    const float *__restrict__ b1, int relu1, const float *__restrict__ w2t,
                                                                    const float *__restrict__ b2, int relu2, const float *__restrict__ w3t,
                                                                    const float *__restrict__ b3, float *__restrict__ out, int out_stride, long limit) {
    pgather_gemm3_compact_body<NB1>(blockIdx.x, o2, o3, n, m, pmat, p_stride, xyz, new_xyz, rowc, rowsrc, total, w1x, b1, relu1, w2t, b2, relu2, w3t, b3, out,
                                    out_stride, limit);
}

template <int NB1>
__global__ __launch_bounds__(256) void pgather_gemm3_compact_pair_kernel(const CompactMlpArgs a0, const CompactMlpArgs a1, const unsigned split, const unsigned total_x) {
    const bool second = blockIdx.x >= split;
    const CompactMlpArgs &a = second ? a1 : a0;
    pgather_gemm3_compact_body<NB1>(second ? blockIdx.x - split : blockIdx.x, a.o2, a.o3, a.n, a.m, a.pmat, a.p_stride, a.xyz, a.new_xyz, a.rowc, a.rowsrc, a.total,
                                    a.w1x, a.b1, a.relu1, a.w2t, a.b2, a.relu2, a.w3t, a.b3, a.out, a.out_stride, a.limit);
}

__device__ __forceinline__ float4 interp3(float w0, const float4 p0, float w1, const float4 p1, float w2, const float4 p2) {
    return make_float4(__builtin_fmaf(w2, p2.x, __builtin_fmaf(w0, p0.x, w1 * p1.x)), __builtin_fmaf(w2, p2.y, __builtin_fmaf(w0, p0.y, w1 * p1.y)),
                       __builtin_fmaf(w2, p2.z, __builtin_fmaf(w0, p0.z, w1 * p1.z)), __builtin_fmaf(w2, p2.w, __builtin_fmaf(w0, p0.w, w1 * p1.w)));
}
__device__ __forceinline__ float4 ld4(const float *p) { return *reinterpret_cast<const float4 *>(p); }
__device__ __forceinline__ void add4(float4 &y, const float4 a) { y.x += a.x; y.y += a.y; y.z += a.z; y.w += a.w; }
__device__ __forceinline__ void fma4(float4 &y, float s, const float4 a) {
    y.x = __builtin_fmaf(s, a.x, y.x); y.y = __builtin_fmaf(s, a.y, y.y); y.z = __builtin_fmaf(s, a.z, y.z); y.w = __builtin_fmaf(s, a.w, y.w);
}
__device__ __forceinline__ void relu4(float4 &y) { y.x = y.x < 0.f ? 0.f : y.x; y.y = y.y < 0.f ? 0.f : y.y; y.z = y.z < 0.f ? 0.f : y.z; y.w = y.w < 0.f ? 0.f : y.w; }

__device__ __forceinline__ float4 qrow_f4(int k, int o, const float *q0, const float *q1, const float *q2, float w0, float w1, float w2,
                                          const float *lrow, const float *srow, int c1, const float *__restrict__ wb, const float *__restrict__ bias, int relu) {
    float4 y = interp3(w0, ld4(q0 + k), w1, ld4(q1 + k), w2, ld4(q2 + k));
    if (lrow) {
        add4(y, ld4(lrow + k));
    } else {
        for (int j = 0; j < c1; ++j) fma4(y, srow[j], ld4(wb + (long)j * o + k));
        if (bias) add4(y, ld4(bias + k));
    }
    if (relu) relu4(y);
    return y;
}

__global__ __launch_bounds__(256) void qinterp_rows_kernel(long rows, int o, int n, int m, const float *__restrict__ q, const int32_t *__restrict__ idx3,
                                                           const float *__restrict__ w3, const float *__restrict__ lin,
                                                           const float *__restrict__ skip, int c1, const float *__restrict__ wb,
                                                           const float *__restrict__ bias, int relu, float *__restrict__ out) {
    const int q4 = o >> 2;
    const long total = rows * q4;
    for (long e = (long)blockIdx.x * 256 + threadIdx.x; e < total; e += (long)gridDim.x * 256) {
        const long r = e / q4;
        const int c4 = (int)(e - r * q4) * 4;
        const float *qb = q + (size_t)(r / n) * m * o;
        *reinterpret_cast<float4 *>(out + r * (long)o + c4) =
            qrow_f4(c4, o, qb + (size_t)idx3[r * 3 + 0] * o, qb + (size_t)idx3[r * 3 + 1] * o, qb + (size_t)idx3[r * 3 + 2] * o, w3[r * 3 + 0], w3[r * 3 + 1],
                    w3[r * 3 + 2], lin ? lin + r * (long)o : nullptr, skip + r * (long)c1, c1, wb, bias, relu);
    }
}

template <int MB, bool PRE>
struct InterpA {
    const float *f0[MB], *f1[MB], *f2[MB], *urow[MB], *lrow[MB];
    float w0[MB], w1[MB], w2[MB];
    int c2, c1, relu_a;
    const float *wb, *b1;
    __device__ __forceinline__ InterpA(long r0, int c2_, int c1_, int n, int m, const float *__restrict__ known_feats, const float *__restrict__ unknown_feats,
                                       const int32_t *__restrict__ idx3, const float *__restrict__ w3, const float *__restrict__ lin,
                                       const float *__restrict__ wb_, const float *__restrict__ b1_, int relu_a_)
        : c2(c2_), c1(c1_), relu_a(relu_a_), wb(wb_), b1(b1_) {
#pragma unroll
        for (int i = 0; i < MB; ++i) {
            const long r = r0 + 64 * i;
            const float *base = known_feats + (size_t)(r / n) * m * c2;
            f0[i] = base + (size_t)idx3[r * 3 + 0] * c2; f1[i] = base + (size_t)idx3[r * 3 + 1] * c2; f2[i] = base + (size_t)idx3[r * 3 + 2] * c2;
            w0[i] = w3[r * 3 + 0]; w1[i] = w3[r * 3 + 1]; w2[i] = w3[r * 3 + 2];
            urow[i] = unknown_feats ? unknown_feats + (size_t)r * c1 : nullptr;
            lrow[i] = (PRE && lin) ? lin + (size_t)r * c2 : nullptr;
        }
    }
    __device__ __forceinline__ float4 operator()(int i, int k) const {
        if (k < c2) {
            if (PRE) return qrow_f4(k, c2, f0[i], f1[i], f2[i], w0[i], w1[i], w2[i], lrow[i], urow[i], c1, wb, b1, relu_a);
            return interp3(w0[i], ld4(f0[i] + k), w1[i], ld4(f1[i] + k), w2[i], ld4(f2[i] + k));
        }
        if (PRE) return f4_zero();
        const int ku = k - c2;
        if (ku + 3 < c1) return ld4(urow[i] + ku);
        float v[4] = {0.f, 0.f, 0.f, 0.f};
#pragma unroll
        for (int q = 0; q < 4; ++q) if (ku + q < c1) v[q] = urow[i][ku + q];
        return make_float4(v[0], v[1], v[2], v[3]);
    }
};

template <int MB, int NB, bool PRE>
__device__ __forceinline__ void interp_gemm_tile(long vb, float (&xs)[2][GP_KT][64 * MB + 1], float (&ws)[2][GP_KT][64 * NB], int c2, int c1, int o_dim, int n, int m, const float *__restrict__ known_feats,
                                                 const float *__restrict__ unknown_feats, const int32_t *__restrict__ idx3, const float *__restrict__ w3,
                                                 const float *__restrict__ wt, const float *__restrict__ bias, int relu, float *__restrict__ out, int tps,
                                                 const float *__restrict__ lin, const float *__restrict__ wb, const float *__restrict__ b1, int relu_a) {
    const Wave w;
    long row_tile;
    int col_tile;
    gg_tile<true>(o_dim / (64 * NB), tps, vb, row_tile, col_tile);
    const long row0 = row_tile * (64 * MB);
    const int col0 = col_tile * (64 * NB);
    const InterpA<MB, PRE> load_a(row0 + (w.tid >> 2), c2, c1, n, m, known_feats, unknown_feats, idx3, w3, lin, wb, b1, relu_a);
    floatx16 acc[MB][NB];
    mfma_k_loop<MB, NB, false>(w, acc, xs, ws, PRE ? c2 : c2 + c1, load_a, wt, o_dim, col0);
#pragma unroll
    for (int i = 0; i < MB; ++i)
#pragma unroll
        for (int j = 0; j < NB; ++j) store_rows(w, acc[i][j], bias, relu, out, o_dim, row0 + sub_row<MB>(w, i), col0 + sub_col<NB, false>(w, j) + w.l32);
}

__global__ __launch_bounds__(256, 8) void interp_gemm_kernel(int c2, int c1, int o_dim, int n, int m, const float *__restrict__ known_feats,
                                                          const float *__restrict__ unknown_feats, const int32_t *__restrict__ idx3,
                                                          const float *__restrict__ w3, const float *__restrict__ wt,
                                                          const float *__restrict__ bias, int relu, float *__restrict__ out, int tps) {
    __shared__ float xs[2][GP_KT][GP_XS];
    __shared__ __attribute__((aligned(16))) float ws[2][GP_KT][64];
    interp_gemm_tile<1, 1, false>(blockIdx.x, xs, ws, c2, c1, o_dim, n, m, known_feats, unknown_feats, idx3, w3, wt, bias, relu, out, tps, nullptr, nullptr,
                                  nullptr, 0);
}

template <int MB, int NB, bool PRE = false>
__global__ __launch_bounds__(256) void interp_gemm_big_kernel(int c2, int c1, int o_dim, int n, int m, const float *__restrict__ known_feats,
                                                              const float *__restrict__ unknown_feats, const int32_t *__restrict__ idx3,
                                                              const float *__restrict__ w3, const float *__restrict__ wt,
                                                              const float *__restrict__ bias, int relu, float *__restrict__ out, int tps,
                                                              const float *__restrict__ lin = nullptr, const float *__restrict__ wb = nullptr,
                                                              const float *__restrict__ b1 = nullptr, int relu_a = 0, long total_tiles = 0) {
    __shared__ float xs[2][GP_KT][64 * MB + 1];
    __shared__ __attribute__((aligned(16))) float ws[2][GP_KT][64 * NB];
    const long n_tiles = total_tiles > 0 ? total_tiles : (long)gridDim.x;
    for (long vb = blockIdx.x; vb < n_tiles; vb += gridDim.x)
        interp_gemm_tile<MB, NB, PRE>(vb, xs, ws, c2, c1, o_dim, n, m, known_feats, unknown_feats, idx3, w3, wt, bias, relu, out, tps, lin, wb, b1, relu_a);
}

}

extern "C" int ws3d_gemm_pool(long rows, int nsample, int k_dim, int o_dim, const float *x_rows, const float *wt,
                              const float *bias, int relu, float *out, int out_stride, const int32_t *gate, long gate_limit, ws3d_stream_t stream) {
    using namespace ws3d;
    const uintptr_t al = reinterpret_cast<uintptr_t>(x_rows) | reinterpret_cast<uintptr_t>(wt);
    if (rows < 0 || (nsample != 16 && nsample != 32) || k_dim <= 0 || (k_dim & 3) || o_dim <= 0 || (o_dim & 63) || (rows & 63) ||
        !x_rows || !wt || !out || out_stride < o_dim || (al & 15)) {
        set_error("ws3d_gemm_pool: unsupported shape (rows=%ld ns=%d k=%d o=%d; rows, o %% 64, k %% 4, ns 16|32)", rows, nsample,
                  k_dim, o_dim);
        return WS3D_E_UNSUPPORTED;
    }
    if (rows == 0) return WS3D_OK;
    const int mb = (rows % 128 == 0 && o_dim % 128 == 0 && (rows / 128) * (o_dim / 128) >= 512) ? 2 : 1;
    const long row_tiles = rows / (64 * mb);
    const int xcd = row_tiles % 8 == 0 ? 1 : 0;
    const dim3 grid((unsigned)((o_dim / (64 * mb)) * row_tiles)), block(256);
    const auto kern = mb == 2 ? (nsample == 16 ? gemm_pool_big_kernel<16, 2, 2> : gemm_pool_big_kernel<32, 2, 2>)
                              : (nsample == 16 ? gemm_pool_big_kernel<16, 1, 1> : gemm_pool_big_kernel<32, 1, 1>);
    hipLaunchKernelGGL(kern, grid, block, 0, as_stream(stream), k_dim, o_dim, x_rows, wt, bias, relu, out, out_stride, xcd, gate, gate_limit);
    return check_launch("ws3d_gemm_pool");
}

extern "C" int ws3d_gather_gemm(int b, int n, int m, int nsample, int c_feat, int o_dim, const float *feats, const float *xyz,
                                const float *new_xyz, const int32_t *nbr, const float *wt, const float *bias, int relu, float *out,
                                ws3d_stream_t stream) {
    using namespace ws3d;
    const long rows = (long)b * m * nsample;
    const uintptr_t al = reinterpret_cast<uintptr_t>(feats) | reinterpret_cast<uintptr_t>(wt);
    if (b < 0 || n <= 0 || m <= 0 || nsample <= 0 || c_feat <= 0 || (c_feat & 3) || o_dim <= 0 || (o_dim & 63) || (rows & 63) || !feats || !xyz ||
        !new_xyz || !nbr || !wt || !out || (al & 15)) {
        set_error("ws3d_gather_gemm: unsupported shape (b=%d n=%d m=%d ns=%d c=%d o=%d; rows, o %% 64, c %% 4)", b, n, m, nsample, c_feat, o_dim);
        return WS3D_E_UNSUPPORTED;
    }
    if (rows == 0) return WS3D_OK;
    constexpr int xcd_env = 1;
    const long per_scene = (long)m * nsample;
    const int tps = (xcd_env && (b & 7) == 0 && per_scene % 64 == 0) ? (int)(per_scene / 64) : 0;
    hipLaunchKernelGGL(gather_gemm_kernel, dim3((unsigned)((o_dim / 64) * (rows / 64))), dim3(256), 0, as_stream(stream), c_feat, o_dim, n, m,
                       nsample, feats, xyz, new_xyz, nbr, wt, bias, relu, out, tps);
    return check_launch("ws3d_gather_gemm");
}

extern "C" int ws3d_interp_gemm(int b, int n, int m, int c2, int c1, int o_dim, const float *known_feats, const float *unknown_feats,
                                const int32_t *idx, const float *weight, const float *wt, const float *bias, int relu, float *out,
                                ws3d_stream_t stream) {
    using namespace ws3d;
    const long rows = (long)b * n;
    const uintptr_t al = reinterpret_cast<uintptr_t>(known_feats) | reinterpret_cast<uintptr_t>(wt) |
                         ((c1 & 3) == 0 ? reinterpret_cast<uintptr_t>(unknown_feats) : 0);
    if (b < 0 || n <= 0 || m <= 0 || c2 <= 0 || (c2 & 3) || c1 < 0 || o_dim <= 0 || (o_dim & 63) || (rows & 63) || !known_feats ||
        (c1 > 0 && !unknown_feats) || !idx || !weight || !wt || !out || (al & 15)) {
        set_error("ws3d_interp_gemm: unsupported shape (b=%d n=%d m=%d c2=%d c1=%d o=%d; rows, o %% 64, c2 %% 4)", b, n, m, c2, c1, o_dim);
        return WS3D_E_UNSUPPORTED;
    }
    if (rows == 0) return WS3D_OK;
    constexpr int xcd_env = 1;
// ... 274 lines not shown
```

ws3d_amd/csrc/gemm_rows.hip:

```cpp
#include "common.h"
#include "split_bf16.h"

namespace ws3d {

typedef unsigned rows_u4 __attribute__((ext_vector_type(4)));
typedef float rows_f4 __attribute__((ext_vector_type(4)));

constexpr int GR_THREADS = 256;
constexpr int GR_TM = 64;
constexpr int GR_KB = 32;
constexpr int GR_FRAG = 1024;
#ifndef WS3D_GR_TALL_MIN_TILES
#define WS3D_GR_TALL_MIN_TILES 512
#endif
constexpr int GR_TALL_MIN_TILES = WS3D_GR_TALL_MIN_TILES;
constexpr int GR_MAX_DIM = 4096;
__host__ __device__ constexpr int gr_tile_rows(int nbt, int mbw) { return nbt == 4 ? 32 * mbw : 64 * mbw; }
__host__ __device__ constexpr int gr_a_stage(int tm) { return tm / 32 * 2 * 3 * GR_FRAG; }
__host__ __device__ constexpr int gr_lds_bytes(int tm) { return 2 * gr_a_stage(tm); }
static_assert(gr_lds_bytes(128) <= 64 * 1024 && gr_lds_bytes(128) * 2 <= 160 * 1024, "inside the default per-workgroup cap, two workgroups per CU");

__global__ __launch_bounds__(256) void gemm_rows_pack_kernel(int K, int N, const float *__restrict__ wt, rows_u4 *__restrict__ pack) {
    const int nb_all = N / 32;
    const long total = (long)(K / GR_KB) * nb_all * 2 * 64;
    for (long i = (long)blockIdx.x * blockDim.x + threadIdx.x; i < total; i += (long)gridDim.x * blockDim.x) {
        const int lane = (int)(i & 63), s = (int)((i >> 6) & 1);
        const long f = i >> 7;
        const int nb = (int)(f % nb_all), kb = (int)(f / nb_all);
        const int col = nb * 32 + (lane & 31), k0 = kb * GR_KB + 16 * s + 8 * (lane >> 5);
        float v[8];
#pragma unroll
        for (int j = 0; j < 8; ++j) v[j] = wt[(long)(k0 + j) * N + col];
        bf16x8 q1, q2, q3;
        split8(v, q1, q2, q3);
        rows_u4 *dst = pack + ((f * 2 + s) * 3) * 64 + lane;
        dst[0] = __builtin_bit_cast(rows_u4, q1);
        dst[64] = __builtin_bit_cast(rows_u4, q2);
        dst[128] = __builtin_bit_cast(rows_u4, q3);
    }
}

template <int NBT, int MBW>
__global__ __launch_bounds__(GR_THREADS, 2) void gemm_rows_kernel(int K, int N, int ntn, const float *__restrict__ a, const rows_u4 *__restrict__ pack,
                                                                  const float *__restrict__ bias, int relu, float *__restrict__ out) {
    extern __shared__ __attribute__((aligned(16))) unsigned char smem_rows[];
    constexpr int TM = gr_tile_rows(NBT, MBW);
    constexpr int UNITS = TM / 64;
    constexpr int STAGE = gr_a_stage(TM);
    const int tid = threadIdx.x, w = tid >> 6, lane = tid & 63, r = lane & 31, h = lane >> 5;
    const int tn = (int)(blockIdx.x % (unsigned)ntn);
    const long tm = blockIdx.x / (unsigned)ntn;
    const int nb_all = N / 32, nkb = K / GR_KB;
    const int nbl = NBT == 4 ? w : (w & 1), mb0 = NBT == 4 ? 0 : (w >> 1) * MBW;

    const int srow = (lane & 7) + 8 * (lane >> 5) + 16 * w, skq = (lane >> 3) & 3;
    const rows_f4 *ap = reinterpret_cast<const rows_f4 *>(a + (tm * TM + srow) * (long)K + 8 * skq);
    const size_t a_unit = (size_t)16 * K;
    const int a_wr = ((srow >> 5) * 2 + (skq >> 1)) * 3 * GR_FRAG + ((skq & 1) * 32 + (srow & 31)) * 16;
    const rows_u4 *wp = pack + (size_t)(tn * NBT + nbl) * 6 * 64 + lane;
    const size_t w_kb = (size_t)nb_all * 6 * 64;

    floatx16 acc[MBW];
#pragma unroll
    for (int m = 0; m < MBW; ++m)
#pragma unroll
        for (int i = 0; i < 16; ++i) acc[m][i] = 0.f;
    rows_u4 wc[6];
#pragma unroll
    for (int i = 0; i < 6; ++i) wc[i] = rows_u4{0u, 0u, 0u, 0u};

    for (int kb = -1; kb < nkb; ++kb) {
        const bool more = kb + 1 < nkb;
        rows_f4 ra[UNITS][2];
        rows_u4 wn[6];
        if (more) {
#pragma unroll
            for (int u = 0; u < UNITS; ++u) {
                ra[u][0] = ap[u * a_unit + (kb + 1) * (GR_KB / 4)];
                ra[u][1] = ap[u * a_unit + (kb + 1) * (GR_KB / 4) + 1];
            }
#pragma unroll
            for (int i = 0; i < 6; ++i) wn[i] = wp[(kb + 1) * w_kb + i * 64];
        }
        if (kb >= 0) {
            const unsigned char *buf = smem_rows + (kb & 1) * STAGE + lane * 16;
#pragma unroll
            for (int s = 0; s < 2; ++s) {
                const bf16x8 w1 = __builtin_bit_cast(bf16x8, wc[3 * s]), w2 = __builtin_bit_cast(bf16x8, wc[3 * s + 1]),
                               w3 = __builtin_bit_cast(bf16x8, wc[3 * s + 2]);
                bf16x8 a1[MBW], a2[MBW], a3[MBW];
#pragma unroll
                for (int m = 0; m < MBW; ++m) {
                    const unsigned char *af = buf + ((mb0 + m) * 2 + s) * 3 * GR_FRAG;
                    a1[m] = *reinterpret_cast<const bf16x8 *>(af);
                    a2[m] = *reinterpret_cast<const bf16x8 *>(af + GR_FRAG);
                    a3[m] = *reinterpret_cast<const bf16x8 *>(af + 2 * GR_FRAG);
                }
                split_mfma6<MBW>(w1, w2, w3, a1, a2, a3, acc);
            }
        }
        if (more) {
            unsigned char *nxt = smem_rows + ((kb + 1) & 1) * STAGE + a_wr;
#pragma unroll
            for (int u = 0; u < UNITS; ++u) {
                const float v[8] = {ra[u][0][0], ra[u][0][1], ra[u][0][2], ra[u][0][3], ra[u][1][0], ra[u][1][1], ra[u][1][2], ra[u][1][3]};
                bf16x8 q1, q2, q3;
                split8(v, q1, q2, q3);
                *reinterpret_cast<bf16x8 *>(nxt + u * 12 * GR_FRAG) = q1;
                *reinterpret_cast<bf16x8 *>(nxt + u * 12 * GR_FRAG + GR_FRAG) = q2;
                *reinterpret_cast<bf16x8 *>(nxt + u * 12 * GR_FRAG + 2 * GR_FRAG) = q3;
            }
#pragma unroll
            for (int i = 0; i < 6; ++i) wc[i] = wn[i];
        }
        __syncthreads();
    }

    const int n0 = (tn * NBT + nbl) * 32 + 4 * h;
    rows_f4 b4[4];
    if (bias) {
#pragma unroll
        for (int g = 0; g < 4; ++g) b4[g] = *reinterpret_cast<const rows_f4 *>(bias + n0 + 8 * g);
    }
#pragma unroll
    for (int m = 0; m < MBW; ++m) {
        float *orow = out + (tm * TM + (mb0 + m) * 32 + r) * (long)N + n0;
#pragma unroll
        for (int g = 0; g < 4; ++g) {
            rows_f4 y;
#pragma unroll
            for (int e = 0; e < 4; ++e) y[e] = acc[m][4 * g + e];
            if (bias) y = y + b4[g];
            if (relu) {
#pragma unroll
                for (int e = 0; e < 4; ++e) y[e] = relu_keep_nan(y[e]);
            }
            *reinterpret_cast<rows_f4 *>(orow + 8 * g) = y;
        }
    }
}

static bool gr_dims_ok(int K, int N) { return K >= GR_KB && K <= GR_MAX_DIM && K % GR_KB == 0 && N >= 64 && N <= GR_MAX_DIM && N % 64 == 0; }

}

extern "C" size_t ws3d_gemm_rows_pack_bytes(int k_dim, int n_dim) {
    return ws3d::gr_dims_ok(k_dim, n_dim) ? (size_t)k_dim * n_dim * 6 : 0;
}

extern "C" int ws3d_gemm_rows_pack(int k_dim, int n_dim, const float *wt, void *pack, ws3d_stream_t stream) {
    using namespace ws3d;
    if (!wt || !pack || (reinterpret_cast<uintptr_t>(pack) & 15) || (reinterpret_cast<uintptr_t>(wt) & 3)) {
        set_error("ws3d_gemm_rows_pack: invalid argument");
        return WS3D_E_INVALID;
    }
    if (!gr_dims_ok(k_dim, n_dim)) {
        set_error("ws3d_gemm_rows_pack: unsupported shape K=%d N=%d (K %% 32, N %% 64, both <= %d)", k_dim, n_dim, GR_MAX_DIM);
        return WS3D_E_UNSUPPORTED;
    }
    const long threads = (long)(k_dim / GR_KB) * (n_dim / 32) * 128;
    hipLaunchKernelGGL(gemm_rows_pack_kernel, dim3((unsigned)((threads + 255) / 256)), dim3(256), 0, as_stream(stream), k_dim, n_dim, wt,
                       static_cast<rows_u4 *>(pack));
    return check_launch("ws3d_gemm_rows_pack");
}

extern "C" int ws3d_gemm_rows_split(long rows, int k_dim, int n_dim, const float *a, const void *pack, const float *bias, int relu, float *out,
                                    ws3d_stream_t stream) {
    using namespace ws3d;
    if (rows < 0 || k_dim <= 0 || n_dim <= 0 || !a || !pack || !out) {
        set_error("ws3d_gemm_rows_split: invalid argument (rows=%ld K=%d N=%d)", rows, k_dim, n_dim);
        return WS3D_E_INVALID;
    }
    const uintptr_t al = reinterpret_cast<uintptr_t>(a) | reinterpret_cast<uintptr_t>(pack) | reinterpret_cast<uintptr_t>(out) | reinterpret_cast<uintptr_t>(bias);
    const int nbt = n_dim % 128 == 0 ? 4 : 2;
    if (!gr_dims_ok(k_dim, n_dim) || rows % GR_TM || (al & 15) || (rows / GR_TM) * (n_dim / (32 * nbt)) > 0x7fffffffL) {
        set_error("ws3d_gemm_rows_split: unsupported shape or alignment (rows=%ld K=%d N=%d; rows %% 64, K %% 32, N %% 64, 16-byte pointers)", rows,
                  k_dim, n_dim);
        return WS3D_E_UNSUPPORTED;
    }
    if (rows == 0) return WS3D_OK;
    const int ntn = n_dim / (32 * nbt);
    const bool tall = nbt == 4 && rows % 128 == 0 && (rows / 128) * ntn >= GR_TALL_MIN_TILES;
    const int tm = tall ? 128 : 64;
    const unsigned grid = (unsigned)((rows / tm) * ntn);
    auto go = [&](auto kern) -> int {
        hipLaunchKernelGGL(kern, dim3(grid), dim3(GR_THREADS), (size_t)gr_lds_bytes(tm), as_stream(stream), k_dim, n_dim, ntn, a,
                           static_cast<const rows_u4 *>(pack), bias, relu ? 1 : 0, out);
        return WS3D_OK;
    };
    if (int rc = nbt == 2 ? go(gemm_rows_kernel<2, 1>) : tall ? go(gemm_rows_kernel<4, 4>) : go(gemm_rows_kernel<4, 2>)) return rc;
    return check_launch("ws3d_gemm_rows_split");
}
```

ws3d_amd/fastpath.py:

```python
from __future__ import annotations

import contextlib
import contextvars

import torch
import torch.nn as nn

from . import compat as _C
from . import nn_blocks, pn2_ops

FUSED_SA_MLP = True
SA1_FROM_LISTS = True
FUSED_GEMM_POOL = True
FUSED_INTERP_GEMM = True
NESTED_FPS = True
GEOMETRY_AHEAD = True
_AHEAD_OVERRIDE = contextvars.ContextVar("ws3d_geometry_ahead", default=None)


@contextlib.contextmanager
def geometry_ahead(on: bool):
    token = _AHEAD_OVERRIDE.set(bool(on))
    try:
        yield
    finally:
        _AHEAD_OVERRIDE.reset(token)


@contextlib.contextmanager
def compact_only_scales(keys):
    token = _COMPACT_ONLY.set(frozenset(keys))
    try:
        yield
    finally:
        _COMPACT_ONLY.reset(token)


def primed_compact_scales(net, pointcloud: torch.Tensor, margin: float = None):
    margin = PRIMED_MARGIN if margin is None else margin
    keys, per_level = set(), {}
    for row in list_fill(net, pointcloud):
        si = per_level.get(row["level"], 0)
        per_level[row["level"]] = si + 1
        if row["fill"] <= margin * COMPACT_MAX_FILL:
            keys.add((row["level"] - 1, si))
    return frozenset(keys)


def _geometry_ahead_now() -> bool:
    v = _AHEAD_OVERRIDE.get()
    return GEOMETRY_AHEAD if v is None else v
GEOMETRY_IN_CAPTURE = False
PER_POINT_L1 = True
COMPACT_MAX_FILL = 0.55
COMPACT_PAIRS = True
PAIR_DISPATCH = "device"
PRIMED_MARGIN = 0.85
_COMPACT_ONLY = contextvars.ContextVar("ws3d_compact_only_scales", default=frozenset())
CHAIN_MLP = True
PAIRED_SCALES = True
MERGED_THREE_NN = True
FUSED_PROLOGUE = True
MERGED_BINNING = True
PER_POINT_FP = True
FUSED_MLP2_ROWS = True
FUSED_HEADS = True
SPLIT_GEMMS = True
FUSED_GATHER_GEMM2 = True
BIN_INPUT_AHEAD = True
FUSED_QINTERP_GEMM_MIN_ROWS = 30000
FUSED_COMPACT3_MAX_LDS = 64 * 1024
FUSED_GATHER_GEMM = True
GRID_MIN_N = 256
DUAL_SCALE_SEARCH = True
NESTED_CHAIN = True
QUERY_CELL_ORDER = True
PARALLEL_SCALES = True
PARALLEL_HEADS = True


def _row_weights(block):
    w, shift, act = block._folded()
    if act is not None and not isinstance(act, nn.ReLU):
        raise NotImplementedError("fast path supports ReLU / no activation only")
    cache = block.__dict__.get("_row_cache")
    if cache is None or cache[0] is not w:
        cache = (w, w.t().contiguous())
        if not torch.cuda.is_current_stream_capturing():
            block.__dict__["_row_cache"] = cache
    return cache[1], shift, act is not None


def _row_weights_xyz_last(block):
    wt, bias, relu = _row_weights(block)
    cache = block.__dict__.get("_row_cache_xyz_last")
    if cache is None or cache[0] is not wt:
        cache = (wt, torch.cat((wt[3:], wt[:3]), dim=0).contiguous())
        if not torch.cuda.is_current_stream_capturing():
            block.__dict__["_row_cache_xyz_last"] = cache
    return cache[1], bias, relu


def _split_rows(block, wt: torch.Tensor, c2: int):
    cache = block.__dict__.get("_split_cache")
    if cache is None or cache[0] is not wt or cache[1] != c2:
        cache = (wt, c2, wt[:c2].contiguous(), wt[c2:].contiguous())
        if not torch.cuda.is_current_stream_capturing():
            block.__dict__["_split_cache"] = cache
    return cache[2], cache[3]


_SPLIT_GEMM_LIBRARY_WINS = frozenset({(512, 1024, 512)})


def _split_gemm_wins(rows: int, k: int, n: int) -> bool:
    return (rows, k, n) not in _SPLIT_GEMM_LIBRARY_WINS


def _split_gemm(x2d: torch.Tensor, holder, key: str, wt: torch.Tensor, bias=None, relu: bool = False):
    if not SPLIT_GEMMS or x2d.dim() != 2 or not _split_gemm_wins(x2d.size(0), wt.size(0), wt.size(1)):
        return None
    packs = holder.__dict__.get("_gemm_rows_packs")
    ent = None if packs is None else packs.get(key)
    if ent is None or ent[0] is not wt:
        if torch.cuda.is_current_stream_capturing():
            return None
        ent = (wt, _C.gemm_rows_pack(wt))
        holder.__dict__.setdefault("_gemm_rows_packs", {})[key] = ent
    if ent[1] is None:
        return None
    return _C.gemm_rows_split(x2d, ent[1], wt.size(1), bias, relu)


def gemm_rows_packs(model):
    return [ent[1] for m in model.modules() for ent in m.__dict__.get("_gemm_rows_packs", {}).values() if ent[1] is not None]


def _layer(x2d: torch.Tensor, block) -> torch.Tensor:
    wt, bias, relu = _row_weights(block)
    y = _split_gemm(x2d, block, "row", wt, bias, relu)
    if y is not None:
        return y
    if bias is None:
        y = torch.mm(x2d, wt)
        return torch.relu_(y) if relu else y
    if relu:
        return torch._addmm_activation(bias, x2d, wt, use_gelu=False)
    return torch.addmm(bias, x2d, wt)


def _blocks(seq):
    return [m for m in seq if isinstance(m, nn_blocks._ConvBlock)]


def mlp_rows(x2d: torch.Tensor, seq, ticket=None) -> torch.Tensor:
    blocks = _blocks(seq)
    if FUSED_MLP2_ROWS and len(blocks) == 2 and x2d.size(1) == 128 and x2d.is_contiguous():
        (w1, b1, r1), (w2, b2, r2) = _row_weights(blocks[0]), _row_weights(blocks[1])
        y = _C.mlp2_rows(x2d, w1, b1, r1, w2, b2, r2, ticket)
        if y is not None:
            return y
    for blk in blocks:
        x2d = _layer(x2d, blk)
    return x2d


def _heads_blob(seq):
    blocks = _blocks(seq)
    if len(blocks) != 2:
        return None
    (w1, b1, r1), (w2, b2, r2) = _row_weights(blocks[0]), _row_weights(blocks[1])
    cache = blocks[0].__dict__.get("_heads_blob")
    if cache is None or cache[0] is not w1 or cache[1] is not b1 or cache[2] is not w2 or cache[3] is not b2:
        cache = (w1, b1, w2, b2, _C.rpn_heads_pack(w1, b1, r1, w2, b2, r2), w2.size(1))
        if not torch.cuda.is_current_stream_capturing():
            blocks[0].__dict__["_heads_blob"] = cache
    return None if cache[4] is None else (cache[4], cache[5])


def heads_blobs(rpn):
    return [blk.__dict__["_heads_blob"][4] for seq in (rpn.rpn_cls_layer, rpn.rpn_reg_layer) for blk in _blocks(seq)[:1]
            if "_heads_blob" in blk.__dict__]


def _fused_heads(rows: torch.Tensor, blobs, which: int, tickets):
    if blobs is None or not all(blobs[i] is not None for i in (0, 1) if which & (1 << i)):
        return None
    (bc, oc), (br, orr) = blobs[0] or (None, 1), blobs[1] or (None, 0)
    if oc != 1 or (which & 2 and orr == 1):
        return None
    return _C.rpn_heads(rows, which, bc, br, orr, tickets, _C.tune("mlp2_wgs") * (2 if which == 3 else 1))


def supported(model) -> bool:
    try:
        for m in model.modules():
            if isinstance(m, nn_blocks._ConvBlock):
                if not m._pointwise or not isinstance(getattr(m, "activation", None), (nn.ReLU, type(None))):
                    return False
        for sa in model.rpn.backbone_net.SA_modules:
            if sa.pool_method != "max_pool" or sa.npoint is None:
                return False
            for g, mlp in zip(sa.groupers, sa.mlps):
                if not isinstance(g, pn2_ops.QueryAndGroup) or any(b.conv.out_channels % 4 for b in _blocks(mlp)):
                    return False
        return True
    except AttributeError:
        return False


def _gather_gemm_ok(sa, grouper, blocks, c_feat: int, B: int) -> bool:
    return (FUSED_GATHER_GEMM and c_feat >= 16 and c_feat % 4 == 0 and grouper.use_xyz and len(blocks) >= 2 and
            blocks[0].conv.out_channels % 64 == 0 and (B * sa.npoint * grouper.nsample) % 64 == 0 and
            (B * sa.npoint * grouper.nsample) // 64 <= 65535)


def _pair_limit(rows: int, dense_available: bool, key=None) -> int:
    if PAIR_DISPATCH != "device" or not dense_available or (key is not None and key in _COMPACT_ONLY.get()):
        return -1
    return max(0, int(COMPACT_MAX_FILL * rows))


@torch.no_grad()
def list_fill(net, pointcloud: torch.Tensor):
    xyz = pointcloud[..., 0:3].contiguous()
    rows = []
    for level, sa in enumerate(net.SA_modules):
        _, new_xyz = (pn2_ops.furthest_point_sample_gather_nested if NESTED_FPS and level >= 1 else pn2_ops.furthest_point_sample_gather)(xyz, sa.npoint)
        srt = pn2_ops.sort_points_x(xyz)
        for g in sa.groupers:
            nbr = _C.ball_query_lists(g.radius, g.nsample, xyz, new_xyz, srt)
            total = _C.compact_pairs(nbr)[2]
            rows.append({"level": level + 1, "n": xyz.size(1), "npoint": sa.npoint, "radius": float(g.radius), "nsample": g.nsample,
                         "distinct_per_list": float(total.item()) / max(nbr.numel() // g.nsample, 1),
                         "fill": float(total.item()) / max(nbr.numel(), 1)})
        xyz = new_xyz
    return rows


class _ZeroArena:

    def __init__(self, numel: int, device, clear: bool = True):
        n = (max(int(numel), 4) + 3) & ~3
        self.buf = (torch.zeros if clear else torch.empty)(n, dtype=torch.float32, device=device)
        self.dirty = not clear
        self.off = 0
        self.fallbacks = 0

    def ensure_clear(self):
        if self.dirty:
            self.buf.zero_()
            self.dirty = False

    def take(self, shape, dtype=torch.float32):
        n = 1
        for d in shape:
            n *= int(d)
        if self.off + n > self.buf.numel():
            self.fallbacks += 1
            self.fallback_shapes = getattr(self, "fallback_shapes", []) + [(tuple(shape), self.off, self.buf.numel())]
            return torch.zeros(shape, dtype=dtype, device=self.buf.device)
        v = self.buf[self.off:self.off + n]
        self.off += (n + 3) & ~3
        return (v if dtype == torch.float32 else v.view(dtype)).view(shape)


LAST_ARENA_FALLBACKS = 0


def _arena_for(net, B: int, device, extra: int = 0, clear: bool = True) -> _ZeroArena:
    n = extra + 64
    if COMPACT_PAIRS:
        for sa in net.SA_modules:
            n += B * sa.npoint * sum(_blocks(mlp)[-1].conv.out_channels for mlp in sa.mlps) + 4
            n += 4 * len(sa.groupers)
        if CHAIN_MLP:
            n += _C.chain_ticket_ints() + 4
    return _ZeroArena(n, device, clear)


class _PairList:
    __slots__ = ("nbr", "pairs")

    def __init__(self, nbr, pairs):
# ... 171 lines not shown
        if isinstance(nbr, _PairList):
            nbr, pairs = nbr.nbr, nbr.pairs
        if nbr is not None:
            wt1, b1, r1 = _row_weights_xyz_last(blocks[0])
            if PER_POINT_L1 and len(blocks) >= 3:
                if pp[0] is None:
                    pp[0] = _per_point_l1(sa, feats, nbrs)
                pmat, offs, w1xs = pp[0]
                o1 = blocks[0].conv.out_channels
                y = None
                wt3, b3, r3 = _row_weights(blocks[-1])
                if pairs is not None and o1 <= 256 and len(blocks) == 3 and r3:
                    wt2, b2, r2 = _row_weights(blocks[1])
                    rows, ns, o3 = nbr.numel(), grouper.nsample, wt3.size(1)
                    dense_ok = (o1 in (64, 128) and (sa.npoint * ns) % 64 == 0 and rows // 64 <= 65535 and o3 % 64 == 0 and
                                wt2.size(1) % 4 == 0 and ns in (16, 32))
                    limit = _pair_limit(rows, dense_ok, (level, si))
                    fused = _C.pgather_gemm3_compact(pmat, offs[si], o1, xyz, new_xyz, pairs, w1xs[si], b1, r1, wt2, b2, r2, wt3, b3, out, col,
                                                     limit=limit, max_lds=FUSED_COMPACT3_MAX_LDS)
                    yc = None if fused else _C.pgather_gemm2_compact(pmat, offs[si], o1, xyz, new_xyz, pairs, w1xs[si], b1, r1, wt2, b2, r2, limit=limit)
                    if fused or (yc is not None and _C.gemm_pool_compact(yc, pairs, wt3, b3, out, col, limit=limit)):
                        if limit >= 0:
                            gate = (pairs[2], limit)
                            yd = _C.pgather_gemm2(pmat, offs[si], o1, xyz, new_xyz, nbr, w1xs[si], b1, r1, wt2, b2, r2, out=yc, gate=gate)
                            if yd is None or not _C.gemm_pool(yd, wt3, b3, r3, ns, out, col, gate=gate):
                                yc = _C.pgather_gemm2_compact(pmat, offs[si], o1, xyz, new_xyz, pairs, w1xs[si], b1, r1, wt2, b2, r2, limit=-1)
                                if yc is None or not _C.gemm_pool_compact(yc, pairs, wt3, b3, out, col, limit=-1):
                                    raise RuntimeError("neither the gated dense nor the ungated compact kernels took the shape")
                        return
                if o1 <= 128:
                    wt2, b2, r2 = _row_weights(blocks[1])
                    y = _C.pgather_gemm2(pmat, offs[si], o1, xyz, new_xyz, nbr, w1xs[si], b1, r1, wt2, b2, r2)
                    rest_pp = blocks[2:-1]
                if y is None:
                    y = _C.pgather_rows(pmat, offs[si], o1, xyz, new_xyz, nbr, w1xs[si], b1, r1)
                    rest_pp = blocks[1:-1]
                if y is not None:
                    for blk in rest_pp:
                        y = _layer(y, blk)
                    wt, bias, relu = _row_weights(blocks[-1])
                    if not (FUSED_GEMM_POOL and _C.gemm_pool(y, wt, bias, relu, grouper.nsample, out, col)):
                        _C.rowmax_rows(_layer(y, blocks[-1]), grouper.nsample, out, col)
                    return
            y = None
            rest = blocks[1:-1]
            if FUSED_GATHER_GEMM2 and len(blocks) >= 3 and blocks[0].conv.out_channels <= 128:
                wt2, b2, r2 = _row_weights(blocks[1])
                y = _C.gather_gemm2(feats, xyz, new_xyz, nbr, wt1, b1, r1, wt2, b2, r2)
                if y is not None:
                    rest = blocks[2:-1]
            if y is None:
                y = _C.gather_gemm(feats, xyz, new_xyz, nbr, wt1, b1, r1)
            if y is not None:
                for blk in rest:
                    y = _layer(y, blk)
                wt, bias, relu = _row_weights(blocks[-1])
                if not (FUSED_GEMM_POOL and _C.gemm_pool(y, wt, bias, relu, grouper.nsample, out, col)):
                    _C.rowmax_rows(_layer(y, blocks[-1]), grouper.nsample, out, col)
                return
        if FUSED_SA_MLP and SA1_FROM_LISTS and feats is not None and feats.size(2) == 1 and grouper.use_xyz and len(blocks) == 3:
            layers = [_row_weights(b) for b in blocks]
            if not COMPACT_PAIRS:
                nbr1 = _C.ball_query_lists(grouper.radius, grouper.nsample, xyz, new_xyz, sorted_xyz)
                if _C.sa_mlp3_pool_lists(xyz, new_xyz, feats, nbr1, layers, out, col):
                    return
            else:
                nbr1, pairs1 = sa1_pairs[si] if si in sa1_pairs else _lists_and_pairs(grouper.radius, grouper.nsample, xyz, new_xyz, sorted_xyz, zeros)
                limit = _pair_limit(nbr1.numel(), layers[2][2] and nbr1.numel() % 32 == 0 and grouper.nsample in (16, 32), (level, si))
                if _C.sa_mlp3_pool_compact(xyz, new_xyz, feats, pairs1, layers, out, col, limit=limit):
                    if limit >= 0 and not _C.sa_mlp3_pool_lists(xyz, new_xyz, feats, nbr1, layers, out, col, gate=(pairs1[2], limit)):
                        if not _C.sa_mlp3_pool_compact(xyz, new_xyz, feats, pairs1, layers, out, col, limit=-1):
                            raise RuntimeError("neither ws3d_sa_mlp3_pool_lists nor the ungated compact kernel took the shape")
                    return
        g = _C.query_and_group_nlc(grouper.radius, grouper.nsample, xyz, new_xyz, feats, grouper.use_xyz, sorted_xyz)
        rows = g.view(-1, g.size(3))
        if not (FUSED_SA_MLP and rows.size(1) == 4 and len(blocks) == 3 and
                _C.sa_mlp3_pool(rows, grouper.nsample, [_row_weights(b) for b in blocks], out, col)):
            y = rows
            for blk in blocks[:-1]:
                y = _layer(y, blk)
            wt, bias, relu = _row_weights(blocks[-1])
            if not (FUSED_GEMM_POOL and _C.gemm_pool(y, wt, bias, relu, grouper.nsample, out, col)):
                _C.rowmax_rows(_layer(y, blocks[-1]), grouper.nsample, out, col)

    def run_paired() -> bool:
        if not (PAIRED_SCALES and COMPACT_PAIRS and PER_POINT_L1 and len(widths) == 2 and all(isinstance(n_, _PairList) for n_ in nbrs)):
            return False
        blk = [_blocks(m_) for m_ in sa.mlps]
        if any(len(b_) != 3 or b_[0].conv.out_channels > 256 for b_ in blk) or blk[0][0].conv.out_channels != blk[1][0].conv.out_channels:
            return False
        if any(_pair_limit(n_.nbr.numel(), True, (level, si_)) != -1 for si_, n_ in enumerate(nbrs)):
            return False
        if pp[0] is None:
            pp[0] = _per_point_l1(sa, feats, nbrs)
        pmat, offs, w1xs = pp[0]
        scales = []
        for si_ in range(2):
            _w1, b1, r1 = _row_weights_xyz_last(blk[si_][0])
            wt2, b2, r2 = _row_weights(blk[si_][1])
            wt3, b3, r3 = _row_weights(blk[si_][2])
            if not r3:
                return False
            scales.append({"pmat": pmat, "col0": offs[si_], "o1": blk[si_][0].conv.out_channels, "xyz": xyz, "new_xyz": new_xyz, "pairs": nbrs[si_].pairs,
                           "w1x": w1xs[si_], "b1": b1, "relu1": r1, "w2t": wt2, "b2": b2, "relu2": r2, "w3t": wt3, "b3": b3, "out2d": out, "col_offset": cols[si_]})
        if (CHAIN_MLP and zeros is not None and all(sc_["o1"] == 64 and sc_["w2t"].size(1) <= 96 and sc_["w3t"].size(1) == 128 for sc_ in scales)
                and _C.chain_mlp3(scales, zeros.take((_C.chain_ticket_ints(),), torch.int32))):
            return True
        if _C.compact_mlp_pair(3, scales, max_lds=FUSED_COMPACT3_MAX_LDS):
            return True
        mids = _C.compact_mlp_pair(2, scales)
        if mids is None:
            return False
        if not _C.compact_mlp_pair(1, scales, mids=mids):
            for sc_, mid in zip(scales, mids):
                if not _C.gemm_pool_compact(mid, sc_["pairs"], sc_["w3t"], sc_["b3"], out, sc_["col_offset"], limit=-1):
                    raise RuntimeError("ws3d_gemm_pool_compact declined a shape ws3d_pgather_gemm2_compact took")
        return True

    if run_paired():
        pass
    elif geo is not None and geo.aux is not None and PARALLEL_SCALES and len(widths) == 2:
        if PER_POINT_L1 and any(n is not None and len(_blocks(m)) >= 3 for n, m in zip(nbrs, sa.mlps)):
            pp[0] = _per_point_l1(sa, feats, nbrs)
        fork = torch.cuda.Event()
        fork.record(geo.main)
        geo.aux.wait_event(fork)
        with torch.cuda.stream(geo.aux):
            run_scale(1)
            join = torch.cuda.Event()
            join.record(geo.aux)
        run_scale(0)
        geo.main.wait_event(join)
    else:
        for si in range(len(widths)):
            run_scale(si)
    return new_xyz, out.view(B, sa.npoint, -1)


def fp_forward(fp, unknown: torch.Tensor, known: torch.Tensor, unknown_feats, known_feats: torch.Tensor, nn3=None, sorted_unknown=None,
               known_xz=None):
    B, n = unknown.size(0), unknown.size(1)
    idx, weight = nn3 if nn3 is not None else _C.three_nn_with_weights(unknown, known, known_xz[0] if known_xz is not None else pn2_ops.sort_points_xz(known),
                                                                        sorted_unknown if QUERY_CELL_ORDER else None)
    c2 = known_feats.size(2)
    c1 = 0 if unknown_feats is None else unknown_feats.size(2)
    blocks = _blocks(fp.mlp)
    if PER_POINT_FP and blocks and blocks[0].conv.out_channels % 4 == 0:
        wt1, b1, r1 = _row_weights(blocks[0])
        wa, wb = _split_rows(blocks[0], wt1, c2)
        m = known_feats.size(1)
        q = _split_gemm(known_feats.reshape(B * m, c2), blocks[0], "wa", wa)
        q = (q if q is not None else torch.mm(known_feats.reshape(B * m, c2), wa)).view(B, m, -1)
        fuse2 = len(blocks) == 2 and B * n >= FUSED_QINTERP_GEMM_MIN_ROWS
        if fuse2:
            wt2, b2, r2 = _row_weights(blocks[1])
        if c1 > 4:
            lin = _split_gemm(unknown_feats.reshape(B * n, c1), blocks[0], "wb", wb, b1)
            if lin is None:
                lin = torch.mm(unknown_feats.reshape(B * n, c1), wb) if b1 is None else torch.addmm(b1, unknown_feats.reshape(B * n, c1), wb)
            y = _C.qinterp_gemm(q, idx, weight, wt2, b2, r2, lin=lin, relu=r1) if fuse2 else None
            if y is not None:
                return y.view(B, n, -1)
            y = _C.qinterp_rows(q, idx, weight, lin=lin, relu=r1)
        else:
            sk = None if c1 == 0 else unknown_feats.contiguous()
            y = _C.qinterp_gemm(q, idx, weight, wt2, b2, r2, skip=sk, wb=wb if c1 else None, bias=b1, relu=r1) if fuse2 else None
            if y is not None:
                return y.view(B, n, -1)
            y = _C.qinterp_rows(q, idx, weight, skip=sk, wb=wb if c1 else None, bias=b1, relu=r1)
        if y is not None:
            for blk in blocks[1:]:
                y = _layer(y, blk)
            return y.view(B, n, -1)
    if FUSED_INTERP_GEMM and blocks and blocks[0].conv.out_channels % 64 == 0 and B * n >= 8192:
        wt1, b1, r1 = _row_weights(blocks[0])
        y = _C.interp_gemm(known_feats.contiguous(), None if unknown_feats is None else unknown_feats.contiguous(), idx, weight, wt1, b1, r1)
        if y is not None:
            for blk in blocks[1:]:
                y = _layer(y, blk)
            return y.view(B, n, -1)
    cat = torch.empty((B, n, c2 + c1), dtype=torch.float32, device=unknown.device)
    _C.three_interpolate_nlc(known_feats, idx, weight, cat)
    if c1:
        cat[:, :, c2:] = unknown_feats
    return mlp_rows(cat.view(B * n, c2 + c1), fp.mlp).view(B, n, -1)


@torch.no_grad()
def backbone_forward(net, pointcloud: torch.Tensor, zeros: _ZeroArena = None):
    if FUSED_PROLOGUE and pointcloud.is_cuda and pointcloud.dim() == 3 and pointcloud.is_contiguous() and pointcloud.size(-1) > 3:
        if zeros is None:
            zeros = _arena_for(net, pointcloud.size(0), pointcloud.device, clear=False)
        xyz, feats = _C.split_points_clear(pointcloud, zeros.buf if zeros.dirty else None)
        zeros.dirty = False
    else:
        xyz = pointcloud[..., 0:3].contiguous()
        feats = pointcloud[..., 3:].contiguous() if pointcloud.size(-1) > 3 else None
        if zeros is None:
            zeros = _arena_for(net, xyz.size(0), xyz.device)
        zeros.ensure_clear()
    ahead = _geometry_ahead_now() and (GEOMETRY_IN_CAPTURE or not torch.cuda.is_current_stream_capturing())
    geo = _Geometry(net, xyz, 0 if feats is None else feats.size(2), zeros) if ahead else None
    l_xyz, l_feats, binned = [xyz], [feats], []
    try:
        sas, chain, pre_grid, pre_xz, nn_pre = list(net.SA_modules), None, {}, {}, {}
        for level, sa in enumerate(sas):
            pre = chain[level - 1][1] if (chain is not None and level >= 1) else None
            nx, nf = sa_forward(sa, l_xyz[-1], l_feats[-1], geo, level, zeros, binned, pre, pre_grid.get(level))
            l_xyz.append(nx)
            l_feats.append(nf)
            if geo is None and level == 0 and NESTED_FPS and NESTED_CHAIN and len(sas) > 1:
                chain = pn2_ops.furthest_point_sample_gather_nested_chain(nx, [s_.npoint for s_ in sas[1:]])
                if MERGED_BINNING:
                    lv = [nx] + [c[1] for c in chain]
                    jobs = [(x_, "grid") for x_ in lv[:-1] if x_.size(1) >= GRID_MIN_N] + [(x_, "xz") for x_ in lv if x_.size(1) >= 256]
                    bufs = iter(_C.sort_points_jobs(jobs) if _C.BQ_FINE_GRID else [])
                    if _C.BQ_FINE_GRID:
                        pre_grid = {k + 1: ((next(bufs),) if x_.size(1) >= GRID_MIN_N else (None,)) for k, x_ in enumerate(lv[:-1])}
                        pre_xz = {k + 1: (next(bufs) if x_.size(1) >= 256 else None) for k, x_ in enumerate(lv)}
                        if MERGED_THREE_NN:
                            allx = [l_xyz[0]] + lv
                            qgrid = {0: binned[0]}
                            qgrid.update({k_: v_[0] for k_, v_ in pre_grid.items()})
                            lvls = [k_ for k_ in range(len(sas)) if pre_xz.get(k_ + 1) is not None and allx[k_ + 1].size(1) <= 4096]
                            got = _C.three_nn_jobs([(allx[k_], allx[k_ + 1], pre_xz[k_ + 1], qgrid.get(k_) if QUERY_CELL_ORDER else None) for k_ in lvls])
                            if got is not None:
                                nn_pre = dict(zip(lvls, got))
        for i in range(-1, -(len(net.FP_modules) + 1), -1):
            lvl = len(l_xyz) + i - 1
            nn3 = nn_pre.get(lvl)
            if geo is not None:
                geo.main.wait_event(geo.nn_ready[lvl])
                nn3 = geo.nn[lvl]
            known_level = len(l_xyz) + i
            l_feats[i - 1] = fp_forward(net.FP_modules[i], l_xyz[i - 1], l_xyz[i], l_feats[i - 1], l_feats[i], nn3, binned[len(l_xyz) + i - 1],
                                        (pre_xz[known_level],) if known_level in pre_xz else None)
    finally:
        if geo is not None:
            geo.release()
    return l_xyz[0], l_feats[0]


@torch.no_grad()
def rpn_forward(model, pts_input: torch.Tensor, defer_reg_join: bool = False) -> dict:
    rpn = model.rpn
    zeros = _arena_for(rpn.backbone_net, pts_input.size(0), pts_input.device, extra=8, clear=not FUSED_PROLOGUE)
    xyz, feats = backbone_forward(rpn.backbone_net, pts_input, zeros)
    B, N, C = feats.shape
    rows = feats.view(B * N, C)
    tickets = zeros.take((2,), torch.int32) if (FUSED_MLP2_ROWS or FUSED_HEADS) else (None, None)
    blobs = (_heads_blob(rpn.rpn_cls_layer), _heads_blob(rpn.rpn_reg_layer)) if FUSED_HEADS else None
    reg_ready = None
    if PARALLEL_HEADS and _geometry_ahead_now() and not torch.cuda.is_current_stream_capturing():
        main = torch.cuda.current_stream(rows.device)
        aux = _side_streams(main)[2]
        fork = torch.cuda.Event()
        fork.record(main)
        aux.wait_event(fork)
        with torch.cuda.stream(aux):
            fused = _fused_heads(rows, blobs, 2, tickets)
            rpn_reg = (fused[1] if fused is not None else mlp_rows(rows, rpn.rpn_reg_layer, tickets[1:2])).view(B, N, -1)
            reg_ready = torch.cuda.Event()
            reg_ready.record(aux)
        rpn_reg.record_stream(main)
        fused = _fused_heads(rows, blobs, 1, tickets)
        rpn_cls = (fused[0] if fused is not None else mlp_rows(rows, rpn.rpn_cls_layer, tickets[0:1])).view(B, N, -1)
        if not defer_reg_join:
            main.wait_event(reg_ready)
            reg_ready = None
    else:
        fused = _fused_heads(rows, blobs, 3, tickets)
        if fused is not None:
            rpn_cls, rpn_reg = fused[0].view(B, N, -1), fused[1].view(B, N, -1)
        else:
            rpn_cls = mlp_rows(rows, rpn.rpn_cls_layer, tickets[0:1]).view(B, N, -1)
            rpn_reg = mlp_rows(rows, rpn.rpn_reg_layer, tickets[1:2]).view(B, N, -1)
    global LAST_ARENA_FALLBACKS
    LAST_ARENA_FALLBACKS = zeros.fallbacks if not zeros.fallbacks else getattr(zeros, "fallback_shapes", zeros.fallbacks)
    out = {"rpn_cls": rpn_cls, "rpn_reg": rpn_reg, "backbone_xyz": xyz,
           "backbone_features": feats.transpose(1, 2),
           "backbone_features_nlc": feats}
    if reg_ready is not None:
        out["rpn_reg_ready"] = reg_ready
    return out
```

Baseline: 6993.

## Fuse three-point interpolation into split-bf16 row GEMM for FP second layer

Factors the split-bf16 MFMA row GEMM tile into a shared header templated on an A-row producer. A new producer builds each A tile on the fly from the interpolated q rows plus lin or skip terms, so the FP module's first layer feeds the packed second-layer GEMM directly. It also adds a wide 256-column tile variant. The goal is to drop the intermediate activation round-trip and use the faster split-GEMM path for FP layers of any size, including those below the old fused-kernel row threshold. In exchange it adds more template instantiations, plus a blacklist for a shape where the new path is expected to lose.

```diff
diff --git a/include/ws3d_ops.h b/include/ws3d_ops.h
--- a/include/ws3d_ops.h
+++ b/include/ws3d_ops.h
@@ -233,6 +233,10 @@
                       const float *skip, int c1, const float *wb, const float *b1, int relu1, const float *w2t, const float *b2, int relu2,
                       float *out, ws3d_stream_t stream);
 
+WS3D_API int ws3d_qinterp_gemm_split(int b, int n, int m, int c, int o_dim, const float *q, const int32_t *idx, const float *weight, const float *lin,
+                            const float *skip, int c1, const float *wb, const float *b1, int relu1, const void *pack, const float *b2, int relu2,
+                            float *out, ws3d_stream_t stream);
+
 
 WS3D_API int ws3d_boxes_overlap_bev(int num_a, const float *boxes_a, int num_b, const float *boxes_b,
                            float *ans, ws3d_stream_t stream);
diff --git a/ws3d_amd/_lib.py b/ws3d_amd/_lib.py
--- a/ws3d_amd/_lib.py
+++ b/ws3d_amd/_lib.py
@@ -66,6 +66,7 @@
     "ws3d_rowmax_rows": (_i, [C.c_long, _i, _i, _vp, _vp, _i, _vp]),
     "ws3d_sa_mlp3_pool": (_i, [C.c_long, _i, _i, _i, _i, _vp, _vp, _vp, _vp, _vp, _vp, _vp, _i, _vp, _i, _vp]),
     "ws3d_qinterp_gemm": (_i, [_i, _i, _i, _i, _i, _vp, _vp, _vp, _vp, _vp, _i, _vp, _vp, _i, _vp, _vp, _i, _vp, _vp]),
+    "ws3d_qinterp_gemm_split": (_i, [_i, _i, _i, _i, _i, _vp, _vp, _vp, _vp, _vp, _i, _vp, _vp, _i, _vp, _vp, _i, _vp, _vp]),
     "ws3d_mlp2_rows": (_i, [C.c_long, _i, _i, _i, _vp, _vp, _vp, _i, _vp, _vp, _i, _vp, _vp, _vp]),
     "ws3d_rpn_heads_blob_bytes": (_sz, [_i]),
     "ws3d_rpn_heads_pack": (_i, [_i, _vp, _vp, _i, _vp, _vp, _i, _vp, _vp]),
diff --git a/ws3d_amd/build.py b/ws3d_amd/build.py
--- a/ws3d_amd/build.py
+++ b/ws3d_amd/build.py
@@ -18,7 +18,7 @@
 def lib_path(dist_mode: int = 0) -> str:
     return LIB if dist_mode == 0 else os.path.join(HERE, "libws3d_hip_dm%d.so" % dist_mode)
 ARCH = "gfx950"
-SOURCES = ["core.hip", "fps.hip", "fps_v3.hip", "fps_bucket.hip", "fps_nested.hip", "ballquery_group.hip", "interpolate.hip", "roipool3d.hip", "iou3d.hip", "proposals.hip", "scatter_det.hip", "sa_mlp.hip", "bn_relu.hip", "gemm_pool.hip", "conv_wgrad.hip", "chain_mlp.hip", "rpn_heads.hip", "gemm_rows.hip", "kitti_eval.hip", "instance_clouds.hip", "click.hip", "stage2.hip", "stage2_loss.hip", "rpn_targets.hip"]
+SOURCES = ["core.hip", "fps.hip", "fps_v3.hip", "fps_bucket.hip", "fps_nested.hip", "ballquery_group.hip", "interpolate.hip", "roipool3d.hip", "iou3d.hip", "proposals.hip", "scatter_det.hip", "sa_mlp.hip", "bn_relu.hip", "gemm_pool.hip", "conv_wgrad.hip", "chain_mlp.hip", "rpn_heads.hip", "gemm_rows.hip", "qinterp_split.hip", "kitti_eval.hip", "instance_clouds.hip", "click.hip", "stage2.hip", "stage2_loss.hip", "rpn_targets.hip"]
 CXXFLAGS = ["-O3", "-std=c++17", "-fPIC", "-ffp-contract=off", "-fno-fast-math",
             "-fvisibility=hidden", "-Wall", "-Wno-unused-function"]
 
diff --git a/ws3d_amd/compat.py b/ws3d_amd/compat.py
--- a/ws3d_amd/compat.py
+++ b/ws3d_amd/compat.py
@@ -531,19 +531,33 @@
     return out
 
 
-def qinterp_gemm(q, idx, weight, w2t, b2, relu2, lin=None, skip=None, wb=None, bias=None, relu=True):
+def qinterp_gemm(q, idx, weight, w2t, b2, relu2, lin=None, skip=None, wb=None, bias=None, relu=True, pack=None, out=None):
     dev = _dev(q, idx, weight, w2t)
     _f32(q, "q"); _i32(idx, "idx"); _f32(weight, "weight"); _f32(w2t, "w2t")
     B, M, C = q.shape
     N = idx.size(1)
     O = w2t.size(1)
     c1 = 0 if skip is None else skip.size(2)
-    if ((B * N) % 64 or C % 16 or O % 128 or w2t.size(0) != C or not q.is_contiguous() or not w2t.is_contiguous() or not idx.is_contiguous() or
+    if ((B * N) % 64 or C % 16 or O % (128 if pack is None else 64) or w2t.size(0) != C or not q.is_contiguous() or not w2t.is_contiguous() or
+            not idx.is_contiguous() or
             not weight.is_contiguous() or (lin is None and c1 > 4) or (lin is not None and (tuple(lin.shape) != (B * N, C) or not lin.is_contiguous())) or
             (lin is None and c1 > 0 and (wb is None or tuple(wb.shape) != (c1, C) or not wb.is_contiguous() or not skip.is_contiguous()))):
         return None
-    out = torch.empty((B * N, O), dtype=torch.float32, device=dev)
-    with _on(dev):
+    if pack is not None and (C % 32 or pack.numel() * pack.element_size() < C * O * 6 or (b2 is not None and (not b2.is_contiguous() or b2.numel() != O)) or
+                             (bias is not None and (not bias.is_contiguous() or bias.numel() != C))):
+        return None
+    if out is None:
+        out = torch.empty((B * N, O), dtype=torch.float32, device=dev)
+    elif tuple(out.shape) != (B * N, O) or out.dtype != torch.float32 or not out.is_contiguous():
+        return None
+    with _on(dev):
+        if pack is not None:
+            rc = _lib.load().ws3d_qinterp_gemm_split(B, N, M, C, O, _p(q), _p(idx), _p(weight), _p(lin), _p(skip), c1, _p(wb), _p(bias), int(bool(relu)),
+                                                     _p(pack), _p(b2), int(bool(relu2)), _p(out), _stream())
+            if rc == _lib.E_UNSUPPORTED:
+                return None
+            check(rc, "qinterp_gemm_split")
+            return out
         check(_lib.load().ws3d_qinterp_gemm(B, N, M, C, O, _p(q), _p(idx), _p(weight), _p(lin), _p(skip), c1, _p(wb), _p(bias), int(bool(relu)), _p(w2t),
                                             _p(b2), int(bool(relu2)), _p(out), _stream()), "qinterp_gemm")
     return out
diff --git a/ws3d_amd/csrc/gemm_pool.hip b/ws3d_amd/csrc/gemm_pool.hip
--- a/ws3d_amd/csrc/gemm_pool.hip
+++ b/ws3d_amd/csrc/gemm_pool.hip
@@ -3,6 +3,7 @@
 #include "common.h"
 #include "compact_pool.h"
 #include "mfma_tile.h"
+#include "qinterp.h"
 
 namespace ws3d {
 
@@ -339,29 +340,6 @@
                                     a.w1x, a.b1, a.relu1, a.w2t, a.b2, a.relu2, a.w3t, a.b3, a.out, a.out_stride, a.limit);
 }
 
-__device__ __forceinline__ float4 interp3(float w0, const float4 p0, float w1, const float4 p1, float w2, const float4 p2) {
-    return make_float4(__builtin_fmaf(w2, p2.x, __builtin_fmaf(w0, p0.x, w1 * p1.x)), __builtin_fmaf(w2, p2.y, __builtin_fmaf(w0, p0.y, w1 * p1.y)),
-                       __builtin_fmaf(w2, p2.z, __builtin_fmaf(w0, p0.z, w1 * p1.z)), __builtin_fmaf(w2, p2.w, __builtin_fmaf(w0, p0.w, w1 * p1.w)));
-}
-__device__ __forceinline__ float4 ld4(const float *p) { return *reinterpret_cast<const float4 *>(p); }
-__device__ __forceinline__ void add4(float4 &y, const float4 a) { y.x += a.x; y.y += a.y; y.z += a.z; y.w += a.w; }
-__device__ __forceinline__ void fma4(float4 &y, float s, const float4 a) {
-    y.x = __builtin_fmaf(s, a.x, y.x); y.y = __builtin_fmaf(s, a.y, y.y); y.z = __builtin_fmaf(s, a.z, y.z); y.w = __builtin_fmaf(s, a.w, y.w);
-}
-__device__ __forceinline__ void relu4(float4 &y) { y.x = y.x < 0.f ? 0.f : y.x; y.y = y.y < 0.f ? 0.f : y.y; y.z = y.z < 0.f ? 0.f : y.z; y.w = y.w < 0.f ? 0.f : y.w; }
-
-__device__ __forceinline__ float4 qrow_f4(int k, int o, const float *q0, const float *q1, const float *q2, float w0, float w1, float w2,
-                                          const float *lrow, const float *srow, int c1, const float *__restrict__ wb, const float *__restrict__ bias, int relu) {
-    float4 y = interp3(w0, ld4(q0 + k), w1, ld4(q1 + k), w2, ld4(q2 + k));
-    if (lrow) {
-        add4(y, ld4(lrow + k));
-    } else {
-        for (int j = 0; j < c1; ++j) fma4(y, srow[j], ld4(wb + (long)j * o + k));
-        if (bias) add4(y, ld4(bias + k));
-    }
-    if (relu) relu4(y);
-    return y;
-}
 
 __global__ __launch_bounds__(256) void qinterp_rows_kernel(long rows, int o, int n, int m, const float *__restrict__ q, const int32_t *__restrict__ idx3,
                                                            const float *__restrict__ w3, const float *__restrict__ lin,
diff --git a/ws3d_amd/csrc/gemm_rows.hip b/ws3d_amd/csrc/gemm_rows.hip
--- a/ws3d_amd/csrc/gemm_rows.hip
+++ b/ws3d_amd/csrc/gemm_rows.hip
@@ -1,24 +1,6 @@
-#include "common.h"
-#include "split_bf16.h"
+#include "gemm_rows_core.h"
 
 namespace ws3d {
-
-typedef unsigned rows_u4 __attribute__((ext_vector_type(4)));
-typedef float rows_f4 __attribute__((ext_vector_type(4)));
-
-constexpr int GR_THREADS = 256;
-constexpr int GR_TM = 64;
-constexpr int GR_KB = 32;
-constexpr int GR_FRAG = 1024;
-#ifndef WS3D_GR_TALL_MIN_TILES
-#define WS3D_GR_TALL_MIN_TILES 512
-#endif
-constexpr int GR_TALL_MIN_TILES = WS3D_GR_TALL_MIN_TILES;
-constexpr int GR_MAX_DIM = 4096;
-__host__ __device__ constexpr int gr_tile_rows(int nbt, int mbw) { return nbt == 4 ? 32 * mbw : 64 * mbw; }
-__host__ __device__ constexpr int gr_a_stage(int tm) { return tm / 32 * 2 * 3 * GR_FRAG; }
-__host__ __device__ constexpr int gr_lds_bytes(int tm) { return 2 * gr_a_stage(tm); }
-static_assert(gr_lds_bytes(128) <= 64 * 1024 && gr_lds_bytes(128) * 2 <= 160 * 1024, "inside the default per-workgroup cap, two workgroups per CU");
 
 __global__ __launch_bounds__(256) void gemm_rows_pack_kernel(int K, int N, const float *__restrict__ wt, rows_u4 *__restrict__ pack) {
     const int nb_all = N / 32;
@@ -43,104 +25,8 @@
 template <int NBT, int MBW>
 __global__ __launch_bounds__(GR_THREADS, 2) void gemm_rows_kernel(int K, int N, int ntn, const float *__restrict__ a, const rows_u4 *__restrict__ pack,
                                                                   const float *__restrict__ bias, int relu, float *__restrict__ out) {
-    extern __shared__ __attribute__((aligned(16))) unsigned char smem_rows[];
-    constexpr int TM = gr_tile_rows(NBT, MBW);
-    constexpr int UNITS = TM / 64;
-    constexpr int STAGE = gr_a_stage(TM);
-    const int tid = threadIdx.x, w = tid >> 6, lane = tid & 63, r = lane & 31, h = lane >> 5;
-    const int tn = (int)(blockIdx.x % (unsigned)ntn);
-    const long tm = blockIdx.x / (unsigned)ntn;
-    const int nb_all = N / 32, nkb = K / GR_KB;
-    const int nbl = NBT == 4 ? w : (w & 1), mb0 = NBT == 4 ? 0 : (w >> 1) * MBW;
-
-    const int srow = (lane & 7) + 8 * (lane >> 5) + 16 * w, skq = (lane >> 3) & 3;
-    const rows_f4 *ap = reinterpret_cast<const rows_f4 *>(a + (tm * TM + srow) * (long)K + 8 * skq);
-    const size_t a_unit = (size_t)16 * K;
-    const int a_wr = ((srow >> 5) * 2 + (skq >> 1)) * 3 * GR_FRAG + ((skq & 1) * 32 + (srow & 31)) * 16;
-    const rows_u4 *wp = pack + (size_t)(tn * NBT + nbl) * 6 * 64 + lane;
-    const size_t w_kb = (size_t)nb_all * 6 * 64;
-
-    floatx16 acc[MBW];
-#pragma unroll
-    for (int m = 0; m < MBW; ++m)
-#pragma unroll
-        for (int i = 0; i < 16; ++i) acc[m][i] = 0.f;
-    rows_u4 wc[6];
-#pragma unroll
-    for (int i = 0; i < 6; ++i) wc[i] = rows_u4{0u, 0u, 0u, 0u};
-
-    for (int kb = -1; kb < nkb; ++kb) {
-        const bool more = kb + 1 < nkb;
-        rows_f4 ra[UNITS][2];
-        rows_u4 wn[6];
-        if (more) {
-#pragma unroll
-            for (int u = 0; u < UNITS; ++u) {
-                ra[u][0] = ap[u * a_unit + (kb + 1) * (GR_KB / 4)];
-                ra[u][1] = ap[u * a_unit + (kb + 1) * (GR_KB / 4) + 1];
-            }
-#pragma unroll
-            for (int i = 0; i < 6; ++i) wn[i] = wp[(kb + 1) * w_kb + i * 64];
-        }
-        if (kb >= 0) {
-            const unsigned char *buf = smem_rows + (kb & 1) * STAGE + lane * 16;
-#pragma unroll
-            for (int s = 0; s < 2; ++s) {
-                const bf16x8 w1 = __builtin_bit_cast(bf16x8, wc[3 * s]), w2 = __builtin_bit_cast(bf16x8, wc[3 * s + 1]),
-                               w3 = __builtin_bit_cast(bf16x8, wc[3 * s + 2]);
-                bf16x8 a1[MBW], a2[MBW], a3[MBW];
-#pragma unroll
-                for (int m = 0; m < MBW; ++m) {
-                    const unsigned char *af = buf + ((mb0 + m) * 2 + s) * 3 * GR_FRAG;
-                    a1[m] = *reinterpret_cast<const bf16x8 *>(af);
-                    a2[m] = *reinterpret_cast<const bf16x8 *>(af + GR_FRAG);
-                    a3[m] = *reinterpret_cast<const bf16x8 *>(af + 2 * GR_FRAG);
-                }
-                split_mfma6<MBW>(w1, w2, w3, a1, a2, a3, acc);
-            }
-        }
-        if (more) {
-            unsigned char *nxt = smem_rows + ((kb + 1) & 1) * STAGE + a_wr;
-#pragma unroll
-            for (int u = 0; u < UNITS; ++u) {
-                const float v[8] = {ra[u][0][0], ra[u][0][1], ra[u][0][2], ra[u][0][3], ra[u][1][0], ra[u][1][1], ra[u][1][2], ra[u][1][3]};
-                bf16x8 q1, q2, q3;
-                split8(v, q1, q2, q3);
-                *reinterpret_cast<bf16x8 *>(nxt + u * 12 * GR_FRAG) = q1;
-                *reinterpret_cast<bf16x8 *>(nxt + u * 12 * GR_FRAG + GR_FRAG) = q2;
-                *reinterpret_cast<bf16x8 *>(nxt + u * 12 * GR_FRAG + 2 * GR_FRAG) = q3;
-            }
-#pragma unroll
-            for (int i = 0; i < 6; ++i) wc[i] = wn[i];
-        }
-        __syncthreads();
-    }
-
-    const int n0 = (tn * NBT + nbl) * 32 + 4 * h;
-    rows_f4 b4[4];
-    if (bias) {
-#pragma unroll
-        for (int g = 0; g < 4; ++g) b4[g] = *reinterpret_cast<const rows_f4 *>(bias + n0 + 8 * g);
-    }
-#pragma unroll
-    for (int m = 0; m < MBW; ++m) {
-        float *orow = out + (tm * TM + (mb0 + m) * 32 + r) * (long)N + n0;
-#pragma unroll
-        for (int g = 0; g < 4; ++g) {
-            rows_f4 y;
-#pragma unroll
-            for (int e = 0; e < 4; ++e) y[e] = acc[m][4 * g + e];
-            if (bias) y = y + b4[g];
-            if (relu) {
-#pragma unroll
-                for (int e = 0; e < 4; ++e) y[e] = relu_keep_nan(y[e]);
-            }
-            *reinterpret_cast<rows_f4 *>(orow + 8 * g) = y;
-        }
-    }
+    gemm_rows_tile<NBT, MBW, RowsContig<gr_tile_rows(NBT, MBW) / 64>>(K, N, ntn, 0, a, pack, bias, relu, out);
 }
-
-static bool gr_dims_ok(int K, int N) { return K >= GR_KB && K <= GR_MAX_DIM && K % GR_KB == 0 && N >= 64 && N <= GR_MAX_DIM && N % 64 == 0; }
 
 }
 
@@ -172,22 +58,18 @@
         return WS3D_E_INVALID;
     }
     const uintptr_t al = reinterpret_cast<uintptr_t>(a) | reinterpret_cast<uintptr_t>(pack) | reinterpret_cast<uintptr_t>(out) | reinterpret_cast<uintptr_t>(bias);
-    const int nbt = n_dim % 128 == 0 ? 4 : 2;
-    if (!gr_dims_ok(k_dim, n_dim) || rows % GR_TM || (al & 15) || (rows / GR_TM) * (n_dim / (32 * nbt)) > 0x7fffffffL) {
+    GrTile t;
+    if (!gr_dims_ok(k_dim, n_dim) || rows % GR_TM || (al & 15) || !gr_tile_choice(rows, n_dim, t)) {
         set_error("ws3d_gemm_rows_split: unsupported shape or alignment (rows=%ld K=%d N=%d; rows %% 64, K %% 32, N %% 64, 16-byte pointers)", rows,
                   k_dim, n_dim);
         return WS3D_E_UNSUPPORTED;
     }
     if (rows == 0) return WS3D_OK;
-    const int ntn = n_dim / (32 * nbt);
-    const bool tall = nbt == 4 && rows % 128 == 0 && (rows / 128) * ntn >= GR_TALL_MIN_TILES;
-    const int tm = tall ? 128 : 64;
-    const unsigned grid = (unsigned)((rows / tm) * ntn);
     auto go = [&](auto kern) -> int {
-        hipLaunchKernelGGL(kern, dim3(grid), dim3(GR_THREADS), (size_t)gr_lds_bytes(tm), as_stream(stream), k_dim, n_dim, ntn, a,
+        hipLaunchKernelGGL(kern, dim3(t.grid), dim3(GR_THREADS), (size_t)gr_lds_bytes(t.tm), as_stream(stream), k_dim, n_dim, t.ntn, a,
                            static_cast<const rows_u4 *>(pack), bias, relu ? 1 : 0, out);
         return WS3D_OK;
     };
-    if (int rc = nbt == 2 ? go(gemm_rows_kernel<2, 1>) : tall ? go(gemm_rows_kernel<4, 4>) : go(gemm_rows_kernel<4, 2>)) return rc;
+    if (int rc = t.nbt == 2 ? go(gemm_rows_kernel<2, 1>) : t.tall ? go(gemm_rows_kernel<4, 4>) : go(gemm_rows_kernel<4, 2>)) return rc;
     return check_launch("ws3d_gemm_rows_split");
 }
diff --git a/ws3d_amd/csrc/gemm_rows_core.h b/ws3d_amd/csrc/gemm_rows_core.h
--- /dev/null
+++ b/ws3d_amd/csrc/gemm_rows_core.h
@@ -0,0 +1,180 @@
+#pragma once
+#include "common.h"
+#include "mfma_tile.h"
+#include "split_bf16.h"
+
+namespace ws3d {
+
+typedef unsigned rows_u4 __attribute__((ext_vector_type(4)));
+typedef float rows_f4 __attribute__((ext_vector_type(4)));
+
+constexpr int GR_THREADS = 256;
+constexpr int GR_TM = 64;
+constexpr int GR_KB = 32;
+constexpr int GR_FRAG = 1024;
+#ifndef WS3D_GR_TALL_MIN_TILES
+#define WS3D_GR_TALL_MIN_TILES 512
+#endif
+constexpr int GR_TALL_MIN_TILES = WS3D_GR_TALL_MIN_TILES;
+constexpr int GR_MAX_DIM = 4096;
+__host__ __device__ constexpr int gr_tile_rows(int nbt, int mbw) { return nbt >= 4 ? 32 * mbw : 64 * mbw; }
+__host__ __device__ constexpr int gr_a_stage(int tm) { return tm / 32 * 2 * 3 * GR_FRAG; }
+__host__ __device__ constexpr int gr_lds_bytes(int tm) { return 2 * gr_a_stage(tm); }
+static_assert(gr_lds_bytes(128) <= 64 * 1024 && gr_lds_bytes(128) * 2 <= 160 * 1024, "inside the default per-workgroup cap, two workgroups per CU");
+
+static inline bool gr_dims_ok(int K, int N) { return K >= GR_KB && K <= GR_MAX_DIM && K % GR_KB == 0 && N >= 64 && N <= GR_MAX_DIM && N % 64 == 0; }
+
+struct GrTile {
+    int nbt, ntn, tm;
+    bool tall;
+    unsigned grid;
+};
+static inline bool gr_tile_choice(long rows, int n_dim, GrTile &t) {
+    t.nbt = n_dim % 128 == 0 ? 4 : 2;
+    t.ntn = n_dim / (32 * t.nbt);
+    if ((rows / GR_TM) * t.ntn > 0x7fffffffL) return false;
+    t.tall = t.nbt == 4 && rows % 128 == 0 && (rows / 128) * t.ntn >= GR_TALL_MIN_TILES;
+    t.tm = t.tall ? 128 : 64;
+    t.grid = (unsigned)((rows / t.tm) * t.ntn);
+    return true;
+}
+
+template <int UNITS>
+struct RowsContig {
+    struct Regs { rows_f4 v[UNITS][2]; };
+    const rows_f4 *ap;
+    size_t a_unit;
+    __device__ __forceinline__ RowsContig(const float *__restrict__ a, long row0, int K, int skq)
+        : ap(reinterpret_cast<const rows_f4 *>(a + row0 * (long)K + 8 * skq)), a_unit((size_t)16 * K) {}
+    __device__ __forceinline__ void fetch(int kb, Regs &g) const {
+#pragma unroll
+        for (int u = 0; u < UNITS; ++u) {
+            g.v[u][0] = ap[u * a_unit + kb * (GR_KB / 4)];
+            g.v[u][1] = ap[u * a_unit + kb * (GR_KB / 4) + 1];
+        }
+    }
+    __device__ __forceinline__ void rows8(const Regs &g, int u, int, float (&v)[8]) const {
+#pragma unroll
+        for (int e = 0; e < 4; ++e) { v[e] = g.v[u][0][e]; v[4 + e] = g.v[u][1][e]; }
+    }
+};
+
+template <int U, int UNITS, class Loader>
+__device__ __forceinline__ void gr_stage_units(const Loader &ld, const typename Loader::Regs &ra, int kb, unsigned char *nxt) {
+    if constexpr (U < UNITS) {
+        float v[8];
+        ld.rows8(ra, U, kb, v);
+        bf16x8 q1, q2, q3;
+        split8(v, q1, q2, q3);
+        *reinterpret_cast<bf16x8 *>(nxt + U * 12 * GR_FRAG) = q1;
+        *reinterpret_cast<bf16x8 *>(nxt + U * 12 * GR_FRAG + GR_FRAG) = q2;
+        *reinterpret_cast<bf16x8 *>(nxt + U * 12 * GR_FRAG + 2 * GR_FRAG) = q3;
+        gr_stage_units<U + 1, UNITS>(ld, ra, kb, nxt);
+    }
+}
+
+template <int NBT, int MBW, class Loader, class Src>
+__device__ __forceinline__ void gemm_rows_tile(int K, int N, int ntn, int tps, const Src src, const rows_u4 *__restrict__ pack,
+                                               const float *__restrict__ bias, int relu, float *__restrict__ out) {
+    extern __shared__ __attribute__((aligned(16))) unsigned char smem_rows[];
+    constexpr int TM = gr_tile_rows(NBT, MBW);
+    constexpr int UNITS = TM / 64;
+    constexpr int STAGE = gr_a_stage(TM);
+    const int tid = threadIdx.x, w = tid >> 6, lane = tid & 63, r = lane & 31, h = lane >> 5;
+    int tn = (int)(blockIdx.x % (unsigned)ntn);
+    long tm = blockIdx.x / (unsigned)ntn;
+    if (tps > 0) gg_tile<true>(ntn, tps, blockIdx.x, tm, tn);
+    const int nb_all = N / 32, nkb = K / GR_KB;
+    constexpr int NCB = NBT == 8 ? 2 : 1;
+    const int nbl = NBT >= 4 ? w : (w & 1), mb0 = NBT >= 4 ? 0 : (w >> 1) * MBW;
+
+    const int srow = (lane & 7) + 8 * (lane >> 5) + 16 * w, skq = (lane >> 3) & 3;
+    const Loader ld(src, tm * TM + srow, K, skq);
+    typedef typename Loader::Regs LoaderRegs;
+    const int a_wr = ((srow >> 5) * 2 + (skq >> 1)) * 3 * GR_FRAG + ((skq & 1) * 32 + (srow & 31)) * 16;
+    const rows_u4 *wp = pack + (size_t)(tn * NBT + nbl) * 6 * 64 + lane;
+    const size_t w_kb = (size_t)nb_all * 6 * 64;
+
+    floatx16 acc[NCB][MBW];
+#pragma unroll
+    for (int c = 0; c < NCB; ++c)
+#pragma unroll
+        for (int m = 0; m < MBW; ++m)
+#pragma unroll
+            for (int i = 0; i < 16; ++i) acc[c][m][i] = 0.f;
+    rows_u4 wc[NCB][6];
+#pragma unroll
+    for (int c = 0; c < NCB; ++c)
+#pragma unroll
+        for (int i = 0; i < 6; ++i) wc[c][i] = rows_u4{0u, 0u, 0u, 0u};
+
+    for (int kb = -1; kb < nkb; ++kb) {
+        const bool more = kb + 1 < nkb;
+        LoaderRegs ra;
+        rows_u4 wn[NCB][6];
+        if (more) {
+            ld.fetch(kb + 1, ra);
+#pragma unroll
+            for (int c = 0; c < NCB; ++c)
+#pragma unroll
+                for (int i = 0; i < 6; ++i) wn[c][i] = wp[(kb + 1) * w_kb + (c * 4 * 6 + i) * 64];
+        }
+        if (kb >= 0) {
+            const unsigned char *buf = smem_rows + (kb & 1) * STAGE + lane * 16;
+#pragma unroll
+            for (int s = 0; s < 2; ++s) {
+                bf16x8 a1[MBW], a2[MBW], a3[MBW];
+#pragma unroll
+                for (int m = 0; m < MBW; ++m) {
+                    const unsigned char *af = buf + ((mb0 + m) * 2 + s) * 3 * GR_FRAG;
+                    a1[m] = *reinterpret_cast<const bf16x8 *>(af);
+                    a2[m] = *reinterpret_cast<const bf16x8 *>(af + GR_FRAG);
+                    a3[m] = *reinterpret_cast<const bf16x8 *>(af + 2 * GR_FRAG);
+                }
+#pragma unroll
+                for (int c = 0; c < NCB; ++c) {
+                    const bf16x8 w1 = __builtin_bit_cast(bf16x8, wc[c][3 * s]), w2 = __builtin_bit_cast(bf16x8, wc[c][3 * s + 1]),
+                                   w3 = __builtin_bit_cast(bf16x8, wc[c][3 * s + 2]);
+                    split_mfma6<MBW>(w1, w2, w3, a1, a2, a3, acc[c]);
+                }
+            }
+        }
+        if (more) {
+            unsigned char *nxt = smem_rows + ((kb + 1) & 1) * STAGE + a_wr;
+            gr_stage_units<0, UNITS>(ld, ra, kb + 1, nxt);
+#pragma unroll
+            for (int c = 0; c < NCB; ++c)
+#pragma unroll
+                for (int i = 0; i < 6; ++i) wc[c][i] = wn[c][i];
+        }
+        __syncthreads();
+    }
+
+#pragma unroll
+    for (int c = 0; c < NCB; ++c) {
+        const int n0 = (tn * NBT + nbl + 4 * c) * 32 + 4 * h;
+        rows_f4 b4[4];
+        if (bias) {
+#pragma unroll
+            for (int g = 0; g < 4; ++g) b4[g] = *reinterpret_cast<const rows_f4 *>(bias + n0 + 8 * g);
+        }
+#pragma unroll
+        for (int m = 0; m < MBW; ++m) {
+            float *orow = out + (tm * TM + (mb0 + m) * 32 + r) * (long)N + n0;
+#pragma unroll
+            for (int g = 0; g < 4; ++g) {
+                rows_f4 y;
+#pragma unroll
+                for (int e = 0; e < 4; ++e) y[e] = acc[c][m][4 * g + e];
+                if (bias) y = y + b4[g];
+                if (relu) {
+#pragma unroll
+                    for (int e = 0; e < 4; ++e) y[e] = relu_keep_nan(y[e]);
+                }
+                *reinterpret_cast<rows_f4 *>(orow + 8 * g) = y;
+            }
+        }
+    }
+}
+
+}
diff --git a/ws3d_amd/csrc/qinterp.h b/ws3d_amd/csrc/qinterp.h
--- /dev/null
+++ b/ws3d_amd/csrc/qinterp.h
@@ -0,0 +1,30 @@
+#pragma once
+#include "common.h"
+
+namespace ws3d {
+
+__device__ __forceinline__ float4 interp3(float w0, const float4 p0, float w1, const float4 p1, float w2, const float4 p2) {
+    return make_float4(__builtin_fmaf(w2, p2.x, __builtin_fmaf(w0, p0.x, w1 * p1.x)), __builtin_fmaf(w2, p2.y, __builtin_fmaf(w0, p0.y, w1 * p1.y)),
+                       __builtin_fmaf(w2, p2.z, __builtin_fmaf(w0, p0.z, w1 * p1.z)), __builtin_fmaf(w2, p2.w, __builtin_fmaf(w0, p0.w, w1 * p1.w)));
+}
+__device__ __forceinline__ float4 ld4(const float *p) { return *reinterpret_cast<const float4 *>(p); }
+__device__ __forceinline__ void add4(float4 &y, const float4 a) { y.x += a.x; y.y += a.y; y.z += a.z; y.w += a.w; }
+__device__ __forceinline__ void fma4(float4 &y, float s, const float4 a) {
+    y.x = __builtin_fmaf(s, a.x, y.x); y.y = __builtin_fmaf(s, a.y, y.y); y.z = __builtin_fmaf(s, a.z, y.z); y.w = __builtin_fmaf(s, a.w, y.w);
+}
+__device__ __forceinline__ void relu4(float4 &y) { y.x = y.x < 0.f ? 0.f : y.x; y.y = y.y < 0.f ? 0.f : y.y; y.z = y.z < 0.f ? 0.f : y.z; y.w = y.w < 0.f ? 0.f : y.w; }
+
+__device__ __forceinline__ float4 qrow_f4(int k, int o, const float *q0, const float *q1, const float *q2, float w0, float w1, float w2,
+                                          const float *lrow, const float *srow, int c1, const float *__restrict__ wb, const float *__restrict__ bias, int relu) {
+    float4 y = interp3(w0, ld4(q0 + k), w1, ld4(q1 + k), w2, ld4(q2 + k));
+    if (lrow) {
+        add4(y, ld4(lrow + k));
+    } else {
+        for (int j = 0; j < c1; ++j) fma4(y, srow[j], ld4(wb + (long)j * o + k));
+        if (bias) add4(y, ld4(bias + k));
+    }
+    if (relu) relu4(y);
+    return y;
+}
+
+}
diff --git a/ws3d_amd/csrc/qinterp_split.hip b/ws3d_amd/csrc/qinterp_split.hip
--- /dev/null
+++ b/ws3d_amd/csrc/qinterp_split.hip
@@ -0,0 +1,119 @@
+#include "gemm_rows_core.h"
+#include "qinterp.h"
+
+namespace ws3d {
+
+#ifndef WS3D_QS_WIDE_MIN_TILES
+#define WS3D_QS_WIDE_MIN_TILES 256
+#endif
+constexpr long QS_WIDE_MIN_TILES = WS3D_QS_WIDE_MIN_TILES;
+
+struct QinterpArgs {
+    const float *q, *weight, *lin, *skip, *wb, *b1;
+    const int32_t *idx;
+    int n, m, c, c1, relu1;
+};
+
+template <int UNITS, bool LIN>
+struct RowsQinterp {
+    struct Regs { rows_f4 p[UNITS][3][2], l[LIN ? UNITS : 1][2]; };
+    static __device__ __forceinline__ rows_f4 ldv(const float *base, unsigned off) {
+        return *reinterpret_cast<const rows_f4 *>(reinterpret_cast<const char *>(base) + off);
+    }
+    static __device__ __forceinline__ float4 f4(const rows_f4 v) { return make_float4(v[0], v[1], v[2], v[3]); }
+    const float *q, *lin, *wb, *b1;
+    unsigned q0[UNITS], q1[UNITS], q2[UNITS], lrow[UNITS];
+    float w0[UNITS], w1[UNITS], w2[UNITS], sk[UNITS][LIN ? 1 : 4];
+    int c, c1, relu1;
+    __device__ __forceinline__ RowsQinterp(const QinterpArgs &a, long row0, int, int skq)
+        : q(a.q + 8 * skq), lin(LIN ? a.lin + 8 * skq : nullptr), wb(a.wb ? a.wb + 8 * skq : nullptr), b1(a.b1 ? a.b1 + 8 * skq : nullptr), c(a.c), c1(a.c1),
+          relu1(a.relu1) {
+#pragma unroll
+        for (int u = 0; u < UNITS; ++u) {
+            const long r = row0 + 64 * u;
+            const long qb = (r / a.n) * a.m;
+            q0[u] = (unsigned)((qb + a.idx[r * 3 + 0]) * a.c * 4); q1[u] = (unsigned)((qb + a.idx[r * 3 + 1]) * a.c * 4); q2[u] = (unsigned)((qb + a.idx[r * 3 + 2]) * a.c * 4);
+            w0[u] = a.weight[r * 3 + 0]; w1[u] = a.weight[r * 3 + 1]; w2[u] = a.weight[r * 3 + 2];
+            lrow[u] = LIN ? (unsigned)(r * a.c * 4) : 0u;
+            if (!LIN) {
+#pragma unroll
+                for (int j = 0; j < 4; ++j) sk[u][j] = j < a.c1 ? a.skip[r * (long)a.c1 + j] : 0.f;
+            }
+        }
+    }
+    __device__ __forceinline__ void fetch(int kb, Regs &g) const {
+        const float *qk = q + kb * GR_KB, *lk = lin + kb * GR_KB;
+#pragma unroll
+        for (int u = 0; u < UNITS; ++u) {
+            g.p[u][0][0] = ldv(qk, q0[u]); g.p[u][0][1] = ldv(qk + 4, q0[u]);
+            g.p[u][1][0] = ldv(qk, q1[u]); g.p[u][1][1] = ldv(qk + 4, q1[u]);
+            g.p[u][2][0] = ldv(qk, q2[u]); g.p[u][2][1] = ldv(qk + 4, q2[u]);
+            if (LIN) { g.l[u][0] = ldv(lk, lrow[u]); g.l[u][1] = ldv(lk + 4, lrow[u]); }
+        }
+    }
+    __device__ __forceinline__ void rows8(const Regs &g, int u, int kb, float (&v)[8]) const {
+        const int k = kb * GR_KB;
+#pragma unroll
+        for (int hh = 0; hh < 2; ++hh) {
+            float4 y = interp3(w0[u], f4(g.p[u][0][hh]), w1[u], f4(g.p[u][1][hh]), w2[u], f4(g.p[u][2][hh]));
+            if (LIN) {
+                add4(y, f4(g.l[LIN ? u : 0][hh]));
+            } else {
+#pragma unroll
+                for (int j = 0; j < 4; ++j)
+                    if (j < c1) fma4(y, sk[u][LIN ? 0 : j], ld4(wb + (long)j * c + k + 4 * hh));
+                if (b1) add4(y, ld4(b1 + k + 4 * hh));
+            }
+            if (relu1) relu4(y);
+            v[4 * hh + 0] = y.x; v[4 * hh + 1] = y.y; v[4 * hh + 2] = y.z; v[4 * hh + 3] = y.w;
+        }
+    }
+};
+
+template <int NBT, int MBW, bool LIN>
+__global__ __launch_bounds__(GR_THREADS, 2) void qinterp_split_kernel(int K, int N, int ntn, int tps, const QinterpArgs a, const rows_u4 *__restrict__ pack,
+                                                                      const float *__restrict__ bias, int relu, float *__restrict__ out) {
+    gemm_rows_tile<NBT, MBW, RowsQinterp<gr_tile_rows(NBT, MBW) / 64, LIN>>(K, N, ntn, tps, a, pack, bias, relu, out);
+}
+
+}
+
+extern "C" int ws3d_qinterp_gemm_split(int b, int n, int m, int c, int o_dim, const float *q, const int32_t *idx, const float *weight, const float *lin,
+                                       const float *skip, int c1, const float *wb, const float *b1, int relu1, const void *pack, const float *b2,
+                                       int relu2, float *out, ws3d_stream_t stream) {
+    using namespace ws3d;
+    if (b < 0 || n <= 0 || m <= 0 || c <= 0 || o_dim <= 0 || c1 < 0 || !q || !idx || !weight || !pack || !out) {
+        set_error("ws3d_qinterp_gemm_split: invalid argument (b=%d n=%d m=%d c=%d o=%d c1=%d)", b, n, m, c, o_dim, c1);
+        return WS3D_E_INVALID;
+    }
+    const long rows = (long)b * n;
+    const uintptr_t al = reinterpret_cast<uintptr_t>(q) | reinterpret_cast<uintptr_t>(lin) | reinterpret_cast<uintptr_t>(wb) | reinterpret_cast<uintptr_t>(b1) |
+                         reinterpret_cast<uintptr_t>(pack) | reinterpret_cast<uintptr_t>(out) | reinterpret_cast<uintptr_t>(b2);
+    GrTile t;
+    const bool fits32 = (long)b * m * c * 4 <= 0xffffffffL && rows * c * 4 <= 0xffffffffL;
+    if (!gr_dims_ok(c, o_dim) || rows % GR_TM || (al & 15) || (!lin && (c1 > 4 || (c1 > 0 && (!skip || !wb)))) || !fits32 || !gr_tile_choice(rows, o_dim, t)) {
+        set_error("ws3d_qinterp_gemm_split: unsupported shape or alignment (b=%d n=%d m=%d c=%d o=%d c1=%d; rows %% 64, c %% 32, o %% 64, lin or c1 <= 4, "
+                  "16-byte pointers)", b, n, m, c, o_dim, c1);
+        return WS3D_E_UNSUPPORTED;
+    }
+    if (rows == 0) return WS3D_OK;
+    const QinterpArgs a{q, weight, lin, lin ? nullptr : skip, lin ? nullptr : wb, lin ? nullptr : b1, idx, n, m, c, lin ? 0 : c1, relu1 ? 1 : 0};
+    if (o_dim % 256 == 0 && (rows / 64) * (o_dim / 256) >= QS_WIDE_MIN_TILES) {
+        t.nbt = 8; t.ntn = o_dim / 256; t.tall = false; t.tm = 64;
+        t.grid = (unsigned)((rows / 64) * t.ntn);
+    }
+    const int tps = (b % 8 == 0 && n % t.tm == 0) ? n / t.tm : 0;
+    auto go = [&](auto kern) -> int {
+        hipLaunchKernelGGL(kern, dim3(t.grid), dim3(GR_THREADS), (size_t)gr_lds_bytes(t.tm), as_stream(stream), c, o_dim, t.ntn, tps, a,
+                           static_cast<const rows_u4 *>(pack), b2, relu2 ? 1 : 0, out);
+        return WS3D_OK;
+    };
+    if (t.nbt == 8) {
+        if (int rc = lin ? go(qinterp_split_kernel<8, 2, true>) : go(qinterp_split_kernel<8, 2, false>)) return rc;
+        return check_launch("ws3d_qinterp_gemm_split");
+    }
+    if (int rc = lin ? (t.nbt == 2 ? go(qinterp_split_kernel<2, 1, true>) : t.tall ? go(qinterp_split_kernel<4, 4, true>) : go(qinterp_split_kernel<4, 2, true>))
+                     : (t.nbt == 2 ? go(qinterp_split_kernel<2, 1, false>) : t.tall ? go(qinterp_split_kernel<4, 4, false>) : go(qinterp_split_kernel<4, 2, false>)))
+        return rc;
+    return check_launch("ws3d_qinterp_gemm_split");
+}
diff --git a/ws3d_amd/fastpath.py b/ws3d_amd/fastpath.py
--- a/ws3d_amd/fastpath.py
+++ b/ws3d_amd/fastpath.py
@@ -69,6 +69,7 @@
 FUSED_GATHER_GEMM2 = True
 BIN_INPUT_AHEAD = True
 FUSED_QINTERP_GEMM_MIN_ROWS = 30000
+FUSED_QINTERP_SPLIT = True
 FUSED_COMPACT3_MAX_LDS = 64 * 1024
 FUSED_GATHER_GEMM = True
 GRID_MIN_N = 256
@@ -117,9 +118,14 @@
     return (rows, k, n) not in _SPLIT_GEMM_LIBRARY_WINS
 
 
-def _split_gemm(x2d: torch.Tensor, holder, key: str, wt: torch.Tensor, bias=None, relu: bool = False):
-    if not SPLIT_GEMMS or x2d.dim() != 2 or not _split_gemm_wins(x2d.size(0), wt.size(0), wt.size(1)):
-        return None
+_QINTERP_SPLIT_LOSES = frozenset({(2048, 512, 512)})
+
+
+def _qinterp_split_wins(rows: int, c: int, o: int) -> bool:
+    return (rows, c, o) not in _QINTERP_SPLIT_LOSES
+
+
+def _gemm_rows_pack(holder, key: str, wt: torch.Tensor):
     packs = holder.__dict__.get("_gemm_rows_packs")
     ent = None if packs is None else packs.get(key)
     if ent is None or ent[0] is not wt:
@@ -127,9 +133,16 @@
             return None
         ent = (wt, _C.gemm_rows_pack(wt))
         holder.__dict__.setdefault("_gemm_rows_packs", {})[key] = ent
-    if ent[1] is None:
+    return ent[1]
+
+
+def _split_gemm(x2d: torch.Tensor, holder, key: str, wt: torch.Tensor, bias=None, relu: bool = False):
+    if not SPLIT_GEMMS or x2d.dim() != 2 or not _split_gemm_wins(x2d.size(0), wt.size(0), wt.size(1)):
         return None
-    return _C.gemm_rows_split(x2d, ent[1], wt.size(1), bias, relu)
+    pack = _gemm_rows_pack(holder, key, wt)
+    if pack is None:
+        return None
+    return _C.gemm_rows_split(x2d, pack, wt.size(1), bias, relu)
 
 
 def gemm_rows_packs(model):
@@ -607,18 +620,29 @@
         q = _split_gemm(known_feats.reshape(B * m, c2), blocks[0], "wa", wa)
         q = (q if q is not None else torch.mm(known_feats.reshape(B * m, c2), wa)).view(B, m, -1)
         fuse2 = len(blocks) == 2 and B * n >= FUSED_QINTERP_GEMM_MIN_ROWS
+        pack2 = None
+        if len(blocks) == 2 and SPLIT_GEMMS and FUSED_QINTERP_SPLIT:
+            wt2, b2, r2 = _row_weights(blocks[1])
+            if _qinterp_split_wins(B * n, wt2.size(0), wt2.size(1)):
+                pack2 = _gemm_rows_pack(blocks[1], "row", wt2)
         if fuse2:
             wt2, b2, r2 = _row_weights(blocks[1])
         if c1 > 4:
             lin = _split_gemm(unknown_feats.reshape(B * n, c1), blocks[0], "wb", wb, b1)
             if lin is None:
                 lin = torch.mm(unknown_feats.reshape(B * n, c1), wb) if b1 is None else torch.addmm(b1, unknown_feats.reshape(B * n, c1), wb)
+            y = _C.qinterp_gemm(q, idx, weight, wt2, b2, r2, lin=lin, relu=r1, pack=pack2) if pack2 is not None else None
+            if y is not None:
+                return y.view(B, n, -1)
             y = _C.qinterp_gemm(q, idx, weight, wt2, b2, r2, lin=lin, relu=r1) if fuse2 else None
             if y is not None:
                 return y.view(B, n, -1)
             y = _C.qinterp_rows(q, idx, weight, lin=lin, relu=r1)
         else:
             sk = None if c1 == 0 else unknown_feats.contiguous()
+            y = _C.qinterp_gemm(q, idx, weight, wt2, b2, r2, skip=sk, wb=wb if c1 else None, bias=b1, relu=r1, pack=pack2) if pack2 is not None else None
+            if y is not None:
+                return y.view(B, n, -1)
             y = _C.qinterp_gemm(q, idx, weight, wt2, b2, r2, skip=sk, wb=wb if c1 else None, bias=b1, relu=r1) if fuse2 else None
             if y is not None:
                 return y.view(B, n, -1)
```

New measurement: 6985 (median of 2 runs). About the same (-0.1%).
